# Atomu2014/deep-ctr

Hardware: AMD Instinct MI355X
Metric: examples/sec (higher is better)
Workload: dtype bf16; 1 GPU; FNN L3 train step: 16 fields, 937670 one-hot dims, k=10, hidden 300/100 tanh, batch 4096 per GPU, Zipf(1.1) ids; per_gpu_batch=4096, global_batch=4096, parallelism=single

## Files before the change

deep-ctr_amd/_capi.py:

```python
import ctypes as C
import os

_HERE = os.path.dirname(os.path.abspath(__file__))
LIB_PATH = os.environ.get("FNN_HIP_LIB") or os.path.join(_HERE, "libfnn_hip.so")

FNN_OK = 0
FNN_ERR_ARG, FNN_ERR_HIP, FNN_ERR_STATE, FNN_ERR_RANGE, FNN_ERR_NOMEM = -1, -2, -3, -4, -5
FNN_PREC_F32, FNN_PREC_BF16, FNN_PREC_BF16X3 = 0, 1, 2
PRECISIONS = {'f32': FNN_PREC_F32, 'bf16': FNN_PREC_BF16, 'bf16x3': FNN_PREC_BF16X3}
FNN_ACT_TANH, FNN_ACT_SIGMOID, FNN_ACT_LINEAR = 0, 1, 2
FNN_MEM_HOST, FNN_MEM_DEVICE = 0, 1
FNN_MODE_FM, FNN_MODE_BAG = 0, 1
FNN_DP_SPARSE_LOCAL, FNN_DP_SPARSE_EXCHANGE = 0, 1
FNN_DP_PAYLOAD_SLABS, FNN_DP_PAYLOAD_BUCKET = 0, 1
FNN_DP_COLLECTIVE_CALLBACK, FNN_DP_COLLECTIVE_P2P = 0, 1
ALLREDUCE_FN = C.CFUNCTYPE(C.c_int, C.c_void_p, C.c_void_p, C.c_int64, C.c_void_p)
ALLGATHER_FN = C.CFUNCTYPE(C.c_int, C.c_void_p, C.c_void_p, C.c_void_p, C.c_int64, C.c_void_p)


class fnn_cfg(C.Structure):
    _fields_ = [("n_fields", C.c_int32), ("k", C.c_int32), ("hidden1", C.c_int32),
                ("hidden2", C.c_int32), ("max_batch", C.c_int32), ("precision", C.c_int32),
                ("act", C.c_int32), ("reg_all", C.c_int32), ("lr", C.c_float),
                ("lambda1", C.c_float), ("lambda_fm", C.c_float), ("device", C.c_int32),
                ("stream", C.c_void_p), ("mode", C.c_int32), ("h0", C.c_int32)]


_vp, _i, _i64, _f = C.c_void_p, C.c_int, C.c_int64, C.c_float

SIGNATURES = {
    "fnn_version": (C.c_char_p, []),
    "fnn_cfg_size": (C.c_uint64, []),
    "fnn_last_error": (C.c_char_p, [_vp]),
    "fnn_scat1_form": (C.c_char_p, []),
    "fnn_scat2_form": (C.c_char_p, []),
    "fnn_create": (_i, [C.POINTER(fnn_cfg), C.POINTER(_vp)]),
    "fnn_destroy": (_i, [_vp]),
    "fnn_set_hparams": (_i, [_vp, _f, _f, _f]),
    "fnn_stream": (_vp, [_vp]),
    "fnn_sync": (_i, [_vp]),
    "fnn_set_table": (_i, [_vp, _vp, _i64, _vp, _f, _i]),
    "fnn_get_table": (_i, [_vp, _vp, _i]),
    "fnn_get_rows": (_i, [_vp, _vp, _i64, _vp, _i]),
    "fnn_set_dense": (_i, [_vp, _i, _vp, _vp, _i]),
    "fnn_get_dense": (_i, [_vp, _i, _vp, _vp, _i]),
    "fnn_set_bag_bias": (_i, [_vp, _vp, _i]),
    "fnn_get_bag_bias": (_i, [_vp, _vp, _i]),
    "fnn_gather": (_i, [_vp, _vp, _i, _vp, _i]),
    "fnn_train_step": (_i, [_vp, _vp, _vp, _i, _vp, _vp, _i, _vp, _vp, _i, C.POINTER(_f)]),
    "fnn_set_shadowed": (_i, [_vp, _vp, _i, _i]),
    "fnn_prefetch_ids": (_i, [_vp, _vp, _i]),
    "fnn_train_step_multi": (_i, [_vp, _i, _vp, _vp, _i, _vp, _vp, _i, _vp, _i, _vp, C.POINTER(_f)]),
    "fnn_dp_unique_id": (_i, [_vp]),
    "fnn_dp_init": (_i, [_vp, _i, _i, _vp, _i]),
    "fnn_dp_init_custom": (_i, [_vp, _i, _i, _vp, _vp, _vp, _i]),
    "fnn_dp_shutdown": (_i, [_vp]),
    "fnn_dp_set_payload": (_i, [_vp, _i]),
    "fnn_dp_p2p_export": (_i, [_vp, _vp, _i]),
    "fnn_dp_p2p_attach": (_i, [_vp, _vp, _i]),
    "fnn_dp_set_collective": (_i, [_vp, _i]),
    "fnn_dp_get_config": (_i, [_vp, C.POINTER(_i), C.POINTER(_i), C.POINTER(_i)]),
    "fnn_dp_p2p_max_wait_us": (_i, [_vp, C.POINTER(C.c_double)]),
    "fnn_step_begin": (_i, [_vp, _vp, _vp, _i, _vp, _vp, _i, _vp, _vp, _i]),
    "fnn_dense_grad_bucket": (_i, [_vp, C.POINTER(_vp), C.POINTER(_i64)]),
    "fnn_step_scatter": (_i, [_vp]),
    "fnn_sparse_grad": (_i, [_vp, C.POINTER(_vp), C.POINTER(_i64)]),
    "fnn_step_scatter_global": (_i, [_vp, _vp, _vp, _i]),
    "fnn_step_end": (_i, [_vp, C.POINTER(_f)]),
# ... 145 lines not shown
```

deep-ctr_amd/csrc/fm_api.hip:

```cpp
#include <hip/hip_runtime.h>

#include <algorithm>
#include <cmath>
#include <cstring>
#include <string>
#include <vector>

#include "../../include/fm_hip.h"
#include "../../include/fnn_hip.h"
#include "sparse_rows.hip.h"
#include "metrics.hip.h"
#include "optim.hip.h"
#include "fm_online.hip.h"
#include "arg_ring.h"

using namespace fnn;

namespace {

thread_local std::string g_fm_err;
inline int rup(int x, int m) { return (x + m - 1) / m * m; }

struct FmArgs {
    const int32_t* ids; const float* y; int B, F, K; const float* table16; int64_t n_rows; const float* b;
// ... 269 lines not shown
    fm_body<NF, WV>(a, (int)blockIdx.x - so.nblk, s_gb);
}

struct FmBiasOpt { int opt; float* sb; float lr, b1, b2, eps; };
__device__ __forceinline__ float fm_opt_step(int opt, float w, float g, float& s0, float& s1, float lr, float b1, float b2, float eps) {
    return opt == FM_OPT_FTRL ? ftrl_step(w, g, s0, s1, lr) : adam_step(w, g, s0, s1, lr, b1, b2, eps);
}

__device__ __forceinline__ void fm_tail_body(float* b, const float* gb_part, int n, float lr, float lambda, const float* loss_t, int Ba, float lscale,
                                             float* loss_out, float* sl, const FmBiasOpt& bo)
{
    float v = strided_sum256(gb_part, n);
    sl[threadIdx.x] = v; __syncthreads();
    for (int o = 128; o > 0; o >>= 1) { if ((int)threadIdx.x < o) sl[threadIdx.x] += sl[threadIdx.x + o]; __syncthreads(); }
    const float gsum = sl[0];
    __syncthreads();
    v = strided_sum256(loss_t, Ba);
    sl[threadIdx.x] = v; __syncthreads();
    for (int o = 128; o > 0; o >>= 1) { if ((int)threadIdx.x < o) sl[threadIdx.x] += sl[threadIdx.x + o]; __syncthreads(); }
    if (threadIdx.x == 0) {
        if (bo.opt) *b = fm_opt_step(bo.opt, *b, gsum + lambda * *b, bo.sb[0], bo.sb[1], bo.lr, bo.b1, bo.b2, bo.eps);
        else *b = *b * (1.0f - lr * lambda) - lr * gsum;
        *loss_out = sl[0] * lscale;
    }
}
__global__ __launch_bounds__(256) void k_fm_scat2_tail(const ScatArgs sa, float* b, const float* gb_part, int n, float lr, float lambda,
                                                       const float* loss_t, int Ba, float lscale, float* loss_out, const FmBiasOpt bo)
{
    __shared__ double s_sum[16][16];
    if (blockIdx.x == 0) { fm_tail_body(b, gb_part, n, lr, lambda, loss_t, Ba, lscale, loss_out, reinterpret_cast<float*>(&s_sum[0][0]), bo); return; }
    if (sa.form2 == SCAT2_WAVE) scat2w_body(sa, (int)blockIdx.x - 1, (int)gridDim.x - 1);
    else scat2_body(sa, (int)blockIdx.x - 1, (int)gridDim.x - 1, s_sum);
}
__global__ __launch_bounds__(256) void k_fm_scat1s(const ScatArgs sa) { scat1h_form<true>(sa, blockIdx.x); }
__global__ __launch_bounds__(256) void k_fm_scat2s_tail(const ScatArgs sa, float* b, const float* gb_part, int n, float lr, float lambda,
                                                        const float* loss_t, int Ba, float lscale, float* loss_out, const FmBiasOpt bo)
{
    __shared__ float s_l[256];
    if (blockIdx.x == 0) { fm_tail_body(b, gb_part, n, lr, lambda, loss_t, Ba, lscale, loss_out, s_l, bo); return; }
    scat2w_form<true>(sa, (int)blockIdx.x - 1, (int)gridDim.x - 1);
}
__global__ __launch_bounds__(256) void k_fm_count_marks(const int* __restrict__ tag_shared, int64_t n_rows, int stamp, unsigned long long* out)
{
    __shared__ int s_c[256];
    int c = 0;
    for (int64_t i = (int64_t)blockIdx.x * 256 + threadIdx.x; i < n_rows; i += (int64_t)gridDim.x * 256) c += tag_shared[i] == stamp;
    s_c[threadIdx.x] = c; __syncthreads();
    for (int o = 128; o > 0; o >>= 1) { if ((int)threadIdx.x < o) s_c[threadIdx.x] += s_c[threadIdx.x + o]; __syncthreads(); }
    if (threadIdx.x == 0 && s_c[0]) atomicAdd(out, (unsigned long long)s_c[0]);
}
__global__ __launch_bounds__(256) void k_fm_scatw1(const ScatArgs sa) { scatw1_body(sa, blockIdx.x); }
__global__ __launch_bounds__(256) void k_fm_scatw2_tail(const ScatArgs sa, float* b, const float* gb_part, int n, float lr, float lambda,
                                                        const float* loss_t, int Ba, float lscale, float* loss_out, const FmBiasOpt bo)
{
    __shared__ double s_w[1024];
    if (blockIdx.x == 0) { fm_tail_body(b, gb_part, n, lr, lambda, loss_t, Ba, lscale, loss_out, reinterpret_cast<float*>(s_w), bo); return; }
    scatw2_body(sa, (int)blockIdx.x - 1, (int)gridDim.x - 1, s_w);
}

struct StepTail { float* b; const float* gb_part; int n; float lr, lambda; const float* loss_t; int Ba; float lscale; float* loss_out; FmBiasOpt bo; };
struct StepPack { float loss; int flag; };
struct StepArg {
    FmArgs a; ScatArgs sa; StepTail t;
    int* own_marks; int own_stamp;
    StepPack* pack;
    int nb1;
    int fcls, scls;
    SortArgs so;
};
__device__ __forceinline__ void step_pick(const StepArg* __restrict__ args, const int ncls, const int mblk, const int first, const int tiles,
                                          int& m, int& tile)
{
    const int lin = (int)blockIdx.x - ncls * mblk;
    m = args[first + lin / tiles].fcls;
    tile = lin % tiles;
    if (tile == 0 && threadIdx.x == 0) *args[m].sa.owner_cnt = 0;
}
template <typename KT, int NF, bool WV>
__global__ __launch_bounds__(256) void k_fm_step_fwd(const StepArg* __restrict__ args, const int ncls, const int mblk, const int first,
                                                     const int tiles)
{
    extern __shared__ __align__(16) unsigned char smem[];
    __shared__ float s_gb[16];
    if ((int)blockIdx.x < ncls * mblk) { const SortArgs so = args[(int)blockIdx.x / mblk].so; sortB_body<KT>(so, (int)blockIdx.x % mblk, smem); return; }
    int m, tile;
    step_pick(args, ncls, mblk, first, tiles, m, tile);
    const FmArgs a = args[m].a;
    fm_body<NF, WV>(a, tile, s_gb);
}
template <typename KT, int L, int NC, bool WV>
__global__ __launch_bounds__(256) void k_fm_step_fwd_wide(const StepArg* __restrict__ args, const int ncls, const int mblk, const int first,
                                                          const int tiles)
{
    extern __shared__ __align__(16) unsigned char smem[];
    __shared__ float s_gb[256 / L];
    if ((int)blockIdx.x < ncls * mblk) { const SortArgs so = args[(int)blockIdx.x / mblk].so; sortB_body<KT>(so, (int)blockIdx.x % mblk, smem); return; }
    int m, tile;
    step_pick(args, ncls, mblk, first, tiles, m, tile);
    const FmArgs a = args[m].a;
    fm_wide_body<L, NC, WV>(a, tile, s_gb);
}
__device__ __forceinline__ void step_copy_marks(const StepArg& g, const ScatArgs& sa, const int blk, const int nblk)
{
    if (!g.own_marks) return;
    const int n = sa.F * sa.N2;
    for (int i = blk * 256 + (int)threadIdx.x; i < n; i += nblk * 256) {
        const int4 r = sa.rec[i];
        if (r.x >= 0 && (i % sa.N2) == r.z && sa.tag_shared[r.x] == sa.stamp) g.own_marks[r.x] = g.own_stamp;
    }
}
template <bool SHARED>
__global__ __launch_bounds__(256) void k_fm_step_scat1(const StepArg* __restrict__ args, const int first)
{
    const int m = args[first + blockIdx.y].scls;
    const int nb1 = args[m].nb1;
    if ((int)blockIdx.x >= nb1) return;
    const ScatArgs sa = args[m].sa;
    if (SHARED) step_copy_marks(args[m], sa, blockIdx.x, nb1);
    scat1h_form<SHARED>(sa, blockIdx.x);
}
__global__ __launch_bounds__(256) void k_fm_step_scatw1(const StepArg* __restrict__ args, const int first)
{
    const int m = args[first + blockIdx.y].scls;
    const int nb1 = args[m].nb1;
    if ((int)blockIdx.x >= nb1) return;
    const ScatArgs sa = args[m].sa;
    step_copy_marks(args[m], sa, blockIdx.x, nb1);
    scatw1_body(sa, blockIdx.x);
}
__device__ __forceinline__ void step_tail(const StepArg& g, float* sl)
{
    const StepTail t = g.t;
    fm_tail_body(t.b, t.gb_part, t.n, t.lr, t.lambda, t.loss_t, t.Ba, t.lscale, t.loss_out, sl, t.bo);
    if (threadIdx.x == 0 && g.pack) {
        const int flag = *static_cast<volatile int*>(g.a.err);
        g.pack->loss = *t.loss_out; g.pack->flag = flag;
        if (flag) *g.a.err = 0;
    }
}
template <bool SHARED>
__global__ __launch_bounds__(256) void k_fm_step_scat2_tail(const StepArg* __restrict__ args, const int first)
{
    __shared__ float s_l[256];
    const int m = args[first + blockIdx.y].scls;
    if (blockIdx.x == 0) { step_tail(args[m], s_l); return; }
    const ScatArgs sa = args[m].sa;
    scat2w_form<SHARED>(sa, (int)blockIdx.x - 1, (int)gridDim.x - 1);
}
__global__ __launch_bounds__(256) void k_fm_step_scatw2_tail(const StepArg* __restrict__ args, const int first)
{
    __shared__ double s_w[1024];
    const int m = args[first + blockIdx.y].scls;
    if (blockIdx.x == 0) { step_tail(args[m], reinterpret_cast<float*>(s_w)); return; }
    const ScatArgs sa = args[m].sa;
    scatw2_body(sa, (int)blockIdx.x - 1, (int)gridDim.x - 1, s_w);
}

__global__ void k_fm_rescale(float* table16, size_t n, float s)
{
    const size_t i = (size_t)blockIdx.x * blockDim.x + threadIdx.x;
    if (i < n) table16[i] *= s;
}

__global__ void k_fm_fill(float* p, size_t n, float v)
{
    const size_t i = (size_t)blockIdx.x * blockDim.x + threadIdx.x;
    if (i < n) p[i] = v;
}

template <bool DENSE_G>
__global__ __launch_bounds__(256) void k_fm_opt_pass(float* __restrict__ table16, float* __restrict__ G, const int* __restrict__ stamp, int step,
                                                     float* __restrict__ s0, float* __restrict__ s1, size_t nk, int K, int rw, float lambda,
                                                     int opt, float lr, float b1, float b2, float eps)
{
    const size_t e0 = ((size_t)blockIdx.x * blockDim.x + threadIdx.x) * 4;
    if (e0 >= nk) return;
    size_t row = e0 / K;
    int c = (int)(e0 - row * K);
    const float4 m4 = *reinterpret_cast<const float4*>(s0 + e0), v4 = *reinterpret_cast<const float4*>(s1 + e0);
    float m[4] = {m4.x, m4.y, m4.z, m4.w}, v[4] = {v4.x, v4.y, v4.z, v4.w}, w[4], g[4];
// ... 5 lines not shown
        off[j] = row * rw + c;
        w[j] = live[j] ? table16[off[j]] : 0.f;
        hit[j] = live[j] && (DENSE_G || stamp[row] == step);
        g[j] = hit[j] ? G[off[j]] : 0.f;
        if (++c == K) { c = 0; ++row; }
    }
#pragma unroll
    for (int j = 0; j < 4; ++j) {
        if (!live[j]) continue;
        w[j] = fm_opt_step(opt, w[j], g[j] + lambda * w[j], m[j], v[j], lr, b1, b2, eps);
        table16[off[j]] = w[j];
        if (hit[j]) G[off[j]] = 0.f;
    }
    *reinterpret_cast<float4*>(s0 + e0) = make_float4(m[0], m[1], m[2], m[3]);
    *reinterpret_cast<float4*>(s1 + e0) = make_float4(v[0], v[1], v[2], v[3]);
}


}

struct fm_handle {
    std::string err; int dev = 0; hipStream_t st = nullptr; bool own_stream = false;
    int F = 0, K = 0, Bmax = 0, K1p = 0;
    bool wide = false;
    int rw = SLOT;
    int* noshare = nullptr;
    float* table16 = nullptr; int64_t n_rows = 0; float* b = nullptr; double scale = 1.0;
    float *gxp = nullptr, *loss_t = nullptr, *gb_part = nullptr, *loss_dev = nullptr; int* err_flag = nullptr;
    RowGroupBufs rg; void* skeys = nullptr;
    double* cpow1 = nullptr; bool key64 = true;
    int opt = FM_OPT_SGD; float beta1 = 0.9f, beta2 = 0.999f, eps = 1e-8f; int64_t t = 0; bool dense_g = false;
    int scat_form = SCAT1_HALF;
    int scat2_form = SCAT2_WAVE;
    int sort_merge4 = 0;
    float *s0 = nullptr, *s1 = nullptr, *sb = nullptr, *G = nullptr; int* stamp = nullptr;
    bool shared = false; int* tag_first = nullptr; int* tag_shared = nullptr; int tag_stamp = 0, step_stamp = 0;
    unsigned long long* mark_cnt = nullptr;
    int64_t online_chunk = 65536; fm_online::Out* online_out = nullptr;
    ArgRing online_ring{sizeof(fm_online::Args), 8 * FM_ONLINE_MAX_MODELS};
    ArgRing step_ring{sizeof(StepArg), 4 * FM_STEP_MAX_MODELS};
    ArgRing eval_ring{sizeof(EvalArg), 4 * FM_EVAL_MAX_MODELS};
    hipEvent_t join = nullptr; StepPack* step_pack = nullptr;
};

#define MHK(h, expr) do { hipError_t e_ = (expr); if (e_ != hipSuccess) { (h)->err = std::string(#expr) + ": " + hipGetErrorString(e_); return FNN_ERR_HIP; } } while (0)
#define MFAIL(h, code, msg) do { (h)->err = (msg); return (code); } while (0)

namespace {

int fold_scale(fm_handle* h)
{
    if (h->scale == 1.0 || !h->table16) return FNN_OK;
    const size_t n = (size_t)h->n_rows * h->rw;
    hipLaunchKernelGGL(k_fm_rescale, dim3((unsigned)((n + 255) / 256)), dim3(256), 0, h->st, h->table16, n, (float)h->scale);
    MHK(h, hipGetLastError());
    h->scale = 1.0;
    return FNN_OK;
}

int alloc_tags(fm_handle* h)
{
    for (int** p : {&h->tag_first, &h->tag_shared}) { if (*p) hipFree(*p); *p = nullptr; }
    h->tag_stamp = h->step_stamp = 0;
    if (!h->shared || !h->table16) return FNN_OK;
    for (int** p : {&h->tag_first, &h->tag_shared}) {
        MHK(h, hipMalloc((void**)p, (size_t)h->n_rows * sizeof(int)));
// ... 135 lines not shown
    const int ex = h->wide ? wide_epb(h) : 16;
    launch_fwd<unsigned>(h, nullptr, predict_args(h, ids, wts, B, p_out, fm_wt_env()), rup(B, ex) / ex);
    MHK(h, hipGetLastError());
    return FNN_OK;
}

struct StepPlan { FmArgs a; ScatArgs sa; StepTail t; int nb1; float lr_step; };
StepPlan plan_step(fm_handle* h, const int32_t* ids, const float* wts, const float* y, int B, float lr, float lambda, int reduce_mean,
                   float* p_out, bool wt, const fm_handle* lead, int stamp, int form1, int form2)
{
    StepPlan p;
    const int F = h->F, ex = h->wide ? wide_epb(h) : 16, Ba = rup(B, ex);
    const bool opt = h->opt != FM_OPT_SGD;
    const float dscale = reduce_mean ? 1.0f / (float)B : 1.0f;
    p.lr_step = lr;
    if (opt) {
        h->t += 1;
        if (h->opt == FM_OPT_ADAM)
            p.lr_step = (float)((double)lr * std::sqrt(1.0 - std::pow((double)h->beta2, (double)h->t)) /
                                (1.0 - std::pow((double)h->beta1, (double)h->t)));
    }
    p.a = FmArgs{ids, y, B, F, h->K, h->table16, h->n_rows, h->b, (float)h->scale, dscale, 1, h->gxp, h->K1p, p_out, h->loss_t,
                 h->gb_part, h->err_flag, wt, opt && !h->dense_g ? h->stamp : nullptr, (int)h->t, h->rw, wts};
    if (!opt) h->scale *= 1.0 - (double)lr * (double)lambda;
    RowGroupBufs rg = h->rg;
    rg.rec = lead->rg.rec;
    p.sa = scat_args(rg, SORT_N, F, h->K, h->gxp, h->K1p, h->cpow1, opt ? -1.0 : (double)lr / h->scale, opt ? h->G : h->table16, h->rw);
    if (h->shared) { p.sa.tag_shared = lead->tag_shared; p.sa.stamp = stamp; }
    else if (h->wide) { p.sa.tag_shared = h->noshare; p.sa.stamp = 1; }
    if (h->wide) {
        p.sa.gxf = h->rw;
        p.nb1 = (F * (SORT_N / WCH) * (h->rw / 4) + 255) / 256;
    } else {
        p.nb1 = scat1_blocks(p.sa, form1);
        p.sa.form2 = form2;
    }
    p.t = StepTail{h->b, h->gb_part, Ba / ex, lr, lambda, h->loss_t, Ba, dscale, h->loss_dev,
                   opt ? FmBiasOpt{h->opt, h->sb, p.lr_step, h->beta1, h->beta2, h->eps} : FmBiasOpt{FM_OPT_SGD, nullptr, 0.f, 0.f, 0.f, 0.f}};
    return p;
}

int fm_step(fm_handle* h, const int32_t* ids, const float* wts, const float* y, int B, float lr, float lambda, int reduce_mean, float* p_out)
{
    const int F = h->F;
    SortArgs so{ids, B, F, h->n_rows, h->rg.rec, h->rg.owner_cnt, 4 * F, h->skeys};
    so.merge4 = h->sort_merge4;
    SortArgs sb = so; sb.nblk = 16 * F;
    set_claim(h, sb);
    const bool own_forms = !h->wide && !h->shared;
    const StepPlan p = plan_step(h, ids, wts, y, B, lr, lambda, reduce_mean, p_out, fm_wt_env(), h, sb.stamp,
                                 own_forms ? h->scat_form : SCAT1_HALF, own_forms ? h->scat2_form : SCAT2_WAVE);
    const StepTail& t = p.t;
    launch_sort_runs(h->st, h->key64, so);
    if (h->key64) launch_fwd<unsigned long long>(h, &sb, p.a, t.n);
    else launch_fwd<unsigned>(h, &sb, p.a, t.n);
#define FM_SCAT(k1, k2_tail) do { \
        hipLaunchKernelGGL(k1, dim3(p.nb1), dim3(256), 0, h->st, p.sa); \
        hipLaunchKernelGGL(k2_tail, dim3(1 + 256), dim3(256), 0, h->st, p.sa, t.b, t.gb_part, t.n, t.lr, t.lambda, t.loss_t, t.Ba, t.lscale, \
                           t.loss_out, t.bo); } while (0)
    if (h->wide) FM_SCAT(k_fm_scatw1, k_fm_scatw2_tail);
    else if (h->shared) FM_SCAT(k_fm_scat1s, k_fm_scat2s_tail);
    else FM_SCAT(k_scat1, k_fm_scat2_tail);
#undef FM_SCAT
    MHK(h, hipGetLastError());
    if (h->opt != FM_OPT_SGD) { launch_opt_pass(h, lambda, p.lr_step); MHK(h, hipGetLastError()); return FNN_OK; }
    if (h->scale < 5.96e-8 || h->scale > 1.0) return fold_scale(h);
    return FNN_OK;
}

void launch_opt_pass(fm_handle* h, float lambda, float lr_step)
{
    const size_t nk = (size_t)h->n_rows * h->K;
    const dim3 grid((unsigned)(((nk + 3) / 4 + 255) / 256));
    if (h->dense_g)
        hipLaunchKernelGGL(k_fm_opt_pass<true>, grid, dim3(256), 0, h->st, h->table16, h->G, h->stamp, (int)h->t, h->s0, h->s1, nk, h->K,
                           h->rw, lambda, h->opt, lr_step, h->beta1, h->beta2, h->eps);
    else
        hipLaunchKernelGGL(k_fm_opt_pass<false>, grid, dim3(256), 0, h->st, h->table16, h->G, h->stamp, (int)h->t, h->s0, h->s1, nk, h->K,
                           h->rw, lambda, h->opt, lr_step, h->beta1, h->beta2, h->eps);
}

int ring_take(fm_handle* h0, ArgRing& r, size_t n, size_t* slot)
{
    MHK(h0, fnn::ring_take(r, n, slot));
    return FNN_OK;
}
int ring_send(fm_handle* h0, ArgRing& r, size_t slot, size_t n)
{
    MHK(h0, fnn::ring_send(r, slot, n, h0->st));
    return FNN_OK;
}

struct GroupCall {
    const char* fn; fm_handle* const* hs; int n, max; fm_handle* h0;
// ... 63 lines not shown
int fm_create(int n_fields, int k, int max_batch, int device, void* stream, fm_handle** out)
{
    if (!out) { g_fm_err = "null argument"; return FNN_ERR_ARG; }
    *out = nullptr;
    if (n_fields < 1 || n_fields > 64 || k < 1 || k > 128 || max_batch < 1 || max_batch > SORT_N) {
        g_fm_err = "need 1 <= n_fields <= 64, 1 <= k <= 128 (rank 0..127), 1 <= max_batch <= 4096"; return FNN_ERR_ARG; }
    int ndev = 0;
    if (hipGetDeviceCount(&ndev) != hipSuccess || ndev <= 0) { g_fm_err = "no HIP device (libfnn_hip.so has no CPU fallback)"; return FNN_ERR_HIP; }
    fm_handle* h = new fm_handle();
    h->dev = device; h->F = n_fields; h->K = k; h->Bmax = max_batch;
    h->wide = k > 16; h->rw = h->wide ? rup(k, 4) : SLOT;
    h->K1p = h->wide ? n_fields * h->rw : rup(n_fields, 16) * SLOT;
    auto fail = [&](int code) { g_fm_err = h->err; fm_destroy(h); return code; };
#define FK(expr) do { hipError_t e2_ = (expr); if (e2_ != hipSuccess) { h->err = std::string(#expr) + ": " + hipGetErrorString(e2_); return fail(FNN_ERR_HIP); } } while (0)
    FK(hipSetDevice(h->dev));
    if (stream) h->st = (hipStream_t)stream; else { FK(hipStreamCreateWithFlags(&h->st, hipStreamNonBlocking)); h->own_stream = true; }
    auto al = [&](void** p, size_t bytes) { hipError_t e = hipMalloc(p, bytes); if (e == hipSuccess) e = hipMemsetAsync(*p, 0, bytes, h->st); return e; };
    const size_t Ba = rup(h->Bmax, 16);
    FK(al((void**)&h->gxp, Ba * h->K1p * 4)); FK(al((void**)&h->loss_t, Ba * 4)); FK(al((void**)&h->gb_part, (Ba / 8) * 4));
    FK(al((void**)&h->loss_dev, 4)); FK(al((void**)&h->b, 4)); FK(al((void**)&h->err_flag, 4)); FK(al((void**)&h->sb, 8));
    FK(al((void**)&h->mark_cnt, 8)); FK(al((void**)&h->online_out, sizeof(fm_online::Out)));
    FK(row_group_alloc(h->rg, h->F, SORT_N, h->wide, h->rw, h->st,  true));
    FK(al(&h->skeys, (size_t)h->F * SORT_N * 8));
    {
        std::vector<double> ones(SORT_N + 1, 1.0);
        FK(hipMalloc((void**)&h->cpow1, ones.size() * 8));
        FK(hipMemcpy(h->cpow1, ones.data(), ones.size() * 8, hipMemcpyHostToDevice));
    }
    FK(hipStreamSynchronize(h->st));
#undef FK
    h->dense_g = getenv("FM_OPT_DENSE_G") && atoi(getenv("FM_OPT_DENSE_G")) == 1;
    h->scat_form = scat1_form_env();
    h->scat2_form = scat2_form_env();
    h->sort_merge4 = sort_merge4_env(0);
    if (const char* e = getenv("FM_ONLINE_CHUNK")) { const long long c = atoll(e); if (c >= 1) h->online_chunk = c; }
    *out = h;
    return FNN_OK;
}

int fm_destroy(fm_handle* h)
{
    if (!h) return FNN_ERR_ARG;
    hipSetDevice(h->dev);
    if (h->st) hipStreamSynchronize(h->st);
    void* ptrs[] = {h->table16, h->b, h->gxp, h->loss_t, h->gb_part, h->loss_dev, h->err_flag, h->skeys, h->cpow1, h->s0, h->s1,
                    h->sb, h->G, h->stamp, h->noshare, h->tag_first, h->tag_shared, h->mark_cnt, h->online_out, h->step_pack};
    for (void* p : ptrs) if (p) hipFree(p);
    for (ArgRing* r : {&h->online_ring, &h->step_ring, &h->eval_ring}) ring_release(*r);
    if (h->join) hipEventDestroy(h->join);
    row_group_free(h->rg);
    if (h->own_stream && h->st) hipStreamDestroy(h->st);
    delete h;
    return FNN_OK;
}

int fm_sync(fm_handle* h)
{
    if (!h) return FNN_ERR_ARG;
    int flag = 0;
    MHK(h, hipMemcpyAsync(&flag, h->err_flag, 4, hipMemcpyDeviceToHost, h->st));
    MHK(h, hipStreamSynchronize(h->st));
    if (flag) { MHK(h, hipMemsetAsync(h->err_flag, 0, 4, h->st)); MFAIL(h, FNN_ERR_RANGE, "feature id outside [-1, n_rows)"); }
    return FNN_OK;
}

int fm_set_table(fm_handle* h, const float* rows, int64_t n_rows)
// ... 250 lines not shown
        if (c == (int)cls.size()) cls.push_back(Cls{hs[m], 0});
        cls_of[m] = c;
    }
    std::vector<int> order;
    for (int c = 0; c < (int)cls.size(); ++c) if (cls[c].lead->key64 == cls[0].lead->key64) order.push_back(c);
    const int nride = (int)order.size();
    for (int c = 0; c < (int)cls.size(); ++c) if (cls[c].lead->key64 != cls[0].lead->key64) order.push_back(c);
    std::vector<SortArgs> sorts(cls.size());
    for (int i = 0; i < (int)order.size(); ++i) {
        Cls& k = cls[order[i]];
        fm_handle* h = k.lead;
        SortArgs so{ids, B, F, h->n_rows, h->rg.rec, h->rg.owner_cnt, 4 * F, h->skeys};
        so.merge4 = h->sort_merge4;
        launch_sort_runs(st, h->key64, so);
        so.nblk = 16 * F;
        if (h->shared) {
            so.tag_first = h->tag_first; so.tag_shared = h->tag_shared;
            so.stamp = k.stamp = on_stream(h, st, [&] { return fm_next_stamp(h); });
        }
        sorts[i] = so;
        a[i].so = so;
    }
    MHK(h0, hipGetLastError());

    const bool wt = fm_wt_env();
    auto lay_of = [](const fm_handle* h) { return !h->wide ? 0 : h->rw <= 64 ? 1 : 2; };
    auto form_of = [](const fm_handle* h) { return h->wide ? 2 : h->shared ? 1 : 0; };
    int fcnt[3] = {0, 0, 0}, scnt[3] = {0, 0, 0}, ffirst[3], sfirst[3], fpos[3], spos[3], nb1max[3] = {0, 0, 0};
    for (int m = 0; m < M; ++m) { ++fcnt[lay_of(hs[m])]; ++scnt[form_of(hs[m])]; }
    ffirst[0] = sfirst[0] = 0;
    for (int c = 1; c < 3; ++c) { ffirst[c] = ffirst[c - 1] + fcnt[c - 1]; sfirst[c] = sfirst[c - 1] + scnt[c - 1]; }
    for (int c = 0; c < 3; ++c) { fpos[c] = ffirst[c]; spos[c] = sfirst[c]; }
    std::vector<float> lr_step(M);
    for (int m = 0; m < M; ++m) {
        fm_handle* h = hs[m];
        const Cls& k = cls[cls_of[m]];
        const StepPlan p = plan_step(h, ids, wts, y, B, lr[m], lambda[m], reduce_mean ? reduce_mean[m] : 0, p_out ? p_out[m] : nullptr, wt,
                                     k.lead, k.stamp, SCAT1_HALF, SCAT2_WAVE);
        a[m].a = p.a; a[m].sa = p.sa; a[m].t = p.t; a[m].nb1 = p.nb1;
        lr_step[m] = p.lr_step;
        a[m].own_marks = nullptr; a[m].own_stamp = 0;
        if (h->shared && h != k.lead) { a[m].own_marks = h->tag_shared; a[m].own_stamp = on_stream(h, st, [&] { return fm_next_stamp(h); }); }
        a[m].pack = pack ? pack + m : nullptr;
        a[fpos[lay_of(h)]++].fcls = m;
        a[spos[form_of(h)]++].scls = m;
        nb1max[form_of(h)] = std::max(nb1max[form_of(h)], p.nb1);
    }
    rc = ring_send(h0, h0->step_ring, slot, (size_t)M);
    if (rc != FNN_OK) return rc;
    for (int i = nride; i < (int)order.size(); ++i) {
        const SortArgs& so = sorts[i];
        if (cls[order[i]].lead->key64) hipLaunchKernelGGL((k_sortB<unsigned long long>), dim3(so.nblk), dim3(256), sort_lds_bytes<unsigned long long>(), st, so);
        else hipLaunchKernelGGL((k_sortB<unsigned>), dim3(so.nblk), dim3(256), sort_lds_bytes<unsigned>(), st, so);
    }
    int ride = nride;
    for (int c = 0; c < 3; ++c) {
        if (!fcnt[c]) continue;
        const int tiles = (B + (c == 2 ? 8 : 16) - 1) / (c == 2 ? 8 : 16);
        if (cls[0].lead->key64) launch_step_fwd<unsigned long long>(st, F, wts != nullptr, c, d, ride, 16 * F, ffirst[c], fcnt[c], tiles);
        else launch_step_fwd<unsigned>(st, F, wts != nullptr, c, d, ride, 16 * F, ffirst[c], fcnt[c], tiles);
        ride = 0;
    }
    MHK(h0, hipGetLastError());
    if (scnt[0]) hipLaunchKernelGGL(k_fm_step_scat1<false>, dim3(nb1max[0], scnt[0]), dim3(256), 0, st, d, sfirst[0]);
    if (scnt[1]) hipLaunchKernelGGL(k_fm_step_scat1<true>, dim3(nb1max[1], scnt[1]), dim3(256), 0, st, d, sfirst[1]);
    if (scnt[2]) hipLaunchKernelGGL(k_fm_step_scatw1, dim3(nb1max[2], scnt[2]), dim3(256), 0, st, d, sfirst[2]);
    if (scnt[0]) hipLaunchKernelGGL(k_fm_step_scat2_tail<false>, dim3(1 + 256, scnt[0]), dim3(256), 0, st, d, sfirst[0]);
    if (scnt[1]) hipLaunchKernelGGL(k_fm_step_scat2_tail<true>, dim3(1 + 256, scnt[1]), dim3(256), 0, st, d, sfirst[1]);
    if (scnt[2]) hipLaunchKernelGGL(k_fm_step_scatw2_tail, dim3(1 + 256, scnt[2]), dim3(256), 0, st, d, sfirst[2]);
    MHK(h0, hipGetLastError());
    for (int m = 0; m < M; ++m) {
        fm_handle* h = hs[m];
        if (h->opt != FM_OPT_SGD) {
            on_stream(h, st, [&] { launch_opt_pass(h, lambda[m], lr_step[m]); return 0; });
            MHK(h0, hipGetLastError());
        } else if (h->scale < 5.96e-8 || h->scale > 1.0) {
            const int rf = on_stream(h, st, [&] { return fold_scale(h); });
            if (rf != FNN_OK) return g.member_failed(rf, h, m);
        }
    }
    rc = g.leave();
    if (rc != FNN_OK || !loss_out) return rc;
    std::vector<StepPack> hp(M);
    MHK(h0, hipMemcpyAsync(hp.data(), pack, (size_t)M * sizeof(StepPack), hipMemcpyDeviceToHost, st));
    MHK(h0, hipStreamSynchronize(st));
    std::string bad;
    for (int m = 0; m < M; ++m) {
        loss_out[m] = hp[m].loss;
        if (hp[m].flag) bad += (bad.empty() ? "" : ", ") + std::to_string(m);
    }
    if (!bad.empty()) return g.refuse(FNN_ERR_RANGE, "feature id outside [-1, n_rows) in model(s) " + bad);
    return FNN_OK;
}

const char* fm_online_form(const fm_handle*) { return "plain"; }

int fm_predict(fm_handle* h, const int32_t* ids, int B, float* p_out) { return fm_predict_w(h, ids, nullptr, B, p_out); }

int fm_predict_w(fm_handle* h, const int32_t* ids, const float* wts, int B, float* p_out)
{
// ... 252 lines not shown
```

deep-ctr_amd/csrc/fnn_api.hip:

```cpp
#include <hip/hip_runtime.h>
#include <rccl/rccl.h>
#include <dlfcn.h>

#include <algorithm>

#include <cmath>
#include <cstdio>
#include <cstdlib>
#include <cstring>
#include <map>
#include <mutex>
#include <string>
#include <vector>

#include "../../include/fnn_hip.h"
#include "fnn_step_kernels.hip.h"
#include "metrics.hip.h"
#include "arg_ring.h"

using namespace fnn;

namespace {

thread_local std::string g_create_err;

struct ProfSlot { std::vector<std::pair<hipEvent_t, hipEvent_t>> ev; double ms = 0; int64_t n = 0; };

inline int rup(int x, int m) { return (x + m - 1) / m * m; }
constexpr int WIDE_XW_MAX = 4096;

struct FnnKnobs {
    int wt_stores = 47;
    int step1_waves = 8;
    bool step1_fixed = true;
    bool fused = true;
    int role_off = 0;
    int splitk = 0;
    int scat2_wgs = 256;
    int wgrad_form = -1;
    int scat_form = SCAT1_HALF;
    int scat2_form = SCAT2_WAVE;
    int sort_merge4 = 1;
};

template <typename... A> struct FnnKernel { void (*fn)(A...) = nullptr; int threads = 0; size_t lds = 0; };
template <typename T> using Step1Kernel = FnnKernel<MlpArgs<T>>;
using Step2Kernel = FnnKernel<SortArgs, WgradArgs, int, int, ScatArgs>;
using Step3Kernel = FnnKernel<SortArgs, TailArgs, ScatArgs>;
template <typename T> using GroupKernel = FnnKernel<const GroupArg<T>*>;
static_assert(sizeof(GroupArg<float>) == sizeof(GroupArg<bf16_t>) && sizeof(GroupArg<float>) == sizeof(GroupArg<bs16_t>), "one argument ring serves every element type");
template <typename T> using GroupPredKernel = FnnKernel<const GroupPredArg<T>*, int, int64_t, int, int64_t, int64_t, int>;
static_assert(sizeof(GroupPredArg<float>) == sizeof(GroupPredArg<bf16_t>) && sizeof(GroupPredArg<float>) == sizeof(GroupPredArg<bs16_t>), "one argument ring serves every element type");

struct FnnPlan {
    int F = 0, K = 0, H1 = 0, H2 = 0, xdim = 0, K1p = 0, H1p = 0, H2p = 0;
    int Bmax = 0, ldT = 0, N2max = 0;
    size_t n1 = 0, n2 = 0, nw12 = 0, nw = 0, nslab = 0;
    bool bf16 = false;
    bool split = false;
    bool bag = false; int rw = SLOT; size_t nbag = 0, off_bag = 0;
    bool wide = false;
    bool strip_shape = false;
    bool strip_ok = false;
    int three_launch_max_B = 0;
    int splitk = 4;
    int wgrad_lds = 0;
    FnnKernel<> step1[2];
    bool key64 = false;
    Step2Kernel step2[2];
    Step3Kernel step3[2];
};

}

// ... 142 lines not shown
}

bool strip_shape_ok(const FnnPlan& p) {
    if (p.wide) return false;
    const int c1 = p.H1p / 64, c2 = p.H2p / 64, cx = p.K1p / 64;
    if (cx == 5) return p.bag && c1 == 5 && c2 == 2;
    return cx == 4 && ((c1 == 5 && c2 == 2) || (c1 == 1 && c2 == 1));
}
int next_stamp(fnn_handle* h, fnn_handle::SortSlot& sl) {
    if (!h->bag) return 0;
    if (h->tag_stamp >= (1 << 25) - 1) {
        hipMemsetAsync(h->tag_first, 0, (size_t)h->n_rows * sizeof(int), h->st);
        for (auto& q : h->slot) hipMemsetAsync(q.tag_shared, 0, (size_t)h->n_rows * sizeof(int), h->st);
        h->tag_stamp = 0;
    }
    sl.stamp = ++h->tag_stamp;
    return sl.stamp;
}
int sort_n2(int B) { int N2 = 256; while (N2 < B) N2 <<= 1; return N2; }
constexpr int GLOBAL_BATCH_MAX = 32768;

template <typename T> WgradArgs make_wgrad_args(fnn_handle* h, int Ba) {
    WgradArgs wa;
    wa.p[0] = WgradProb{h->xpT, h->dl1T, h->slab, h->K1p / 64, h->H1p / 64, h->H1p};
    wa.p[1] = WgradProb{h->d1T, h->dl2T, h->slab + h->n1, h->H1p / 64, h->H2p / 64, h->H2p};
    wa.p[2] = WgradProb{h->d2T, h->dl3T, h->slab + h->nw12, h->H2p / 64, 1, 64};
    wa.p[3] = WgradProb{h->dlxT, h->onesT, h->slab + h->off_bag, h->bag ? h->K1p / 64 : 0, 1, 64};
    wa.ldT = h->ldT; wa.klen = Ba / h->splitk; wa.zstride = h->nslab;
    return wa;
}
int wgrad_blocks(const WgradArgs& wa) {
    return wa.p[0].mt * wa.p[0].nt + wa.p[1].mt * wa.p[1].nt + wa.p[2].mt * wa.p[2].nt + wa.p[3].mt * wa.p[3].nt;
}
ScatArgs make_scat_args(fnn_handle* h, const fnn_handle::SortSlot& sl, int N2) {
    ScatArgs sa = scat_args(sl, N2, h->F, h->K, h->gxp, h->K1p, h->cpow_dev, (double)h->cfg.lr, h->table16, h->rw);
    sa.tag_shared = sl.tag_shared; sa.stamp = sl.stamp; sa.form2 = h->kn.scat2_form;
    return sa;
}
template <typename T> MlpArgs<T> make_mlp_args(fnn_handle* h, const int32_t* ids, const float* y, int B,
                                                const uint8_t* m1, const uint8_t* m2, bool train, float* p_out) {
    return MlpArgs<T>{ids, y ? y : h->loss_t, B, h->F, h->K, h->table16, h->n_rows, h->w0,
                      (const T*)h->w1, (const T*)h->w1t, (const T*)h->w2, (const T*)h->w2t, h->master + h->nw12,
                      m1 ? m1 : h->ones_u8, m2 ? m2 : h->ones_u8, h->cfg.act, train ? ACT_TANH : h->cfg.act,
                      h->H1, h->H2, train ? 1 : 0,
                      (T*)h->xpT, (T*)h->d1T, (T*)h->d2T, (T*)h->dl1T, (T*)h->dl2T, (T*)h->dl3T, h->ldT,
                      h->gxp, p_out, h->loss_t, h->err_flag, h->bb0, h->rw, (T*)h->dlxT, nullptr, h->kn.wt_stores};
}
template <typename T> Step1Kernel<T> step1_sel(const FnnPlan& p, const FnnKnobs& kn, bool train)
{
#define STEP1(C1, C2, CX, BAG, NW, ...) Step1Kernel<T>{k_step1<T, C1, C2, CX, BAG, NW, ##__VA_ARGS__>, 64 * NW, mlp_lds_bytes<T, C1, C2, CX>(BAG, p.F, NW)}
    const bool big = p.H1p / 64 == 5, x5 = p.K1p / 64 == 5;
    if (big && kn.step1_waves == 8) {
        if (x5) return STEP1(5, 2, 5, true, 8);
        if (p.bag) return STEP1(5, 2, 4, true, 8);
        if constexpr (std::is_same<T, bf16_t>::value)
            if (kn.step1_fixed && train && kn.wt_stores == 47 && ((8 * p.F + 15) >> 4) * 32 <= 512) return STEP1(5, 2, 4, false, 8, 47);
        return STEP1(5, 2, 4, false, 8);
    }
    if (x5) return STEP1(5, 2, 5, true, 4);
    if (p.bag) return big ? STEP1(5, 2, 4, true, 4) : STEP1(1, 1, 4, true, 4);
    return big ? STEP1(5, 2, 4, false, 4) : STEP1(1, 1, 4, false, 4);
#undef STEP1
}
template <typename T> Step2Kernel step2_sel(bool key64, bool m4, bool wgrad_lds)
{
#define STEP2(WF) (key64 ? (m4 ? Step2Kernel{k_step2<T, unsigned long long, true, WF>, 256, lds} : Step2Kernel{k_step2<T, unsigned long long, false, WF>, 256, lds}) \
                         : (m4 ? Step2Kernel{k_step2<T, unsigned, true, WF>, 256, lds} : Step2Kernel{k_step2<T, unsigned, false, WF>, 256, lds}))
    const size_t lds = key64 ? sortA_lds_bytes<unsigned long long>(m4) : sortA_lds_bytes<unsigned>(m4);
    if constexpr (sizeof(T) == 2) if (wgrad_lds) return STEP2(WGRAD_LDS);
    return STEP2(WGRAD_DIRECT);
#undef STEP2
}
template <typename T> Step3Kernel step3_sel(bool key64, bool m4, bool update)
{
#define STEP3(KT, LDS) (m4 ? (update ? Step3Kernel{k_step3<T, true, KT, true>, 256, LDS} : Step3Kernel{k_step3<T, false, KT, true>, 256, LDS}) \
                           : (update ? Step3Kernel{k_step3<T, true, KT, false>, 256, LDS} : Step3Kernel{k_step3<T, false, KT, false>, 256, LDS}))
    return key64 ? STEP3(unsigned long long, sort_lds_bytes<unsigned long long>()) : STEP3(unsigned, sort_lds_bytes<unsigned>());
#undef STEP3
}
template <typename T> GroupKernel<T> gstep1_sel(const FnnPlan& p, const FnnKnobs& kn)
{
#define GSTEP1(C1, C2, NW, WTF) GroupKernel<T>{k_gstep1<T, C1, C2, 4, NW, WTF>, 64 * NW, mlp_lds_bytes<T, C1, C2, 4>(false, p.F, NW)}
    const bool big = p.H1p / 64 == 5;
    if (big && kn.step1_waves == 8) {
        if constexpr (std::is_same<T, bf16_t>::value)
            if (kn.step1_fixed && kn.wt_stores == 47 && ((8 * p.F + 15) >> 4) * 32 <= 512) return GSTEP1(5, 2, 8, 47);
        return GSTEP1(5, 2, 8, -1);
    }
    return big ? GSTEP1(5, 2, 4, -1) : GSTEP1(1, 1, 4, -1);
#undef GSTEP1
}
template <typename T> GroupPredKernel<T> gpredict_sel(const FnnPlan& p, const FnnKnobs& kn)
{
#define GPREDICT(C1, C2, NW) GroupPredKernel<T>{k_gpredict<T, C1, C2, 4, NW>, 64 * NW, mlp_lds_bytes<T, C1, C2, 4>(false, p.F, NW)}
    const bool big = p.H1p / 64 == 5;
    if (big && kn.step1_waves == 8) return GPREDICT(5, 2, 8);
    return big ? GPREDICT(5, 2, 4) : GPREDICT(1, 1, 4);
#undef GPREDICT
}
template <typename T> GroupKernel<T> gstep2_sel(bool key64, bool m4, bool wgrad_lds)
{
#define GSTEP2(WF) (key64 ? (m4 ? GroupKernel<T>{k_gstep2<T, unsigned long long, true, WF>, 256, lds} : GroupKernel<T>{k_gstep2<T, unsigned long long, false, WF>, 256, lds}) \
                          : (m4 ? GroupKernel<T>{k_gstep2<T, unsigned, true, WF>, 256, lds} : GroupKernel<T>{k_gstep2<T, unsigned, false, WF>, 256, lds}))
    const size_t lds = key64 ? sortA_lds_bytes<unsigned long long>(m4) : sortA_lds_bytes<unsigned>(m4);
    if constexpr (sizeof(T) == 2) if (wgrad_lds) return GSTEP2(WGRAD_LDS);
    return GSTEP2(WGRAD_DIRECT);
#undef GSTEP2
}
template <typename T> GroupKernel<T> gstep3_sel(bool key64, bool m4)
{
#define GSTEP3(KT) (m4 ? GroupKernel<T>{k_gstep3<T, KT, true>, 256, sort_lds_bytes<KT>()} : GroupKernel<T>{k_gstep3<T, KT, false>, 256, sort_lds_bytes<KT>()})
    return key64 ? GSTEP3(unsigned long long) : GSTEP3(unsigned);
#undef GSTEP3
}
template <typename T> void plan_step1(fnn_handle* h)
{
    for (int train = 0; train < 2; ++train) {
        const Step1Kernel<T> k = step1_sel<T>(*h, h->kn, train != 0);
        h->step1[train] = {reinterpret_cast<void (*)()>(k.fn), k.threads, k.lds};
    }
}
template <typename T> void plan_keys(fnn_handle* h, bool key64)
{
    h->key64 = key64;
    for (int i = 0; i < 2; ++i) {
        h->step2[i] = step2_sel<T>(key64, h->kn.sort_merge4 != 0, i && h->wgrad_lds);
        h->step3[i] = step3_sel<T>(key64, h->kn.sort_merge4 != 0, i != 0);
    }
}

template <typename T> void launch_step1(fnn_handle* h, int nmlp, const MlpArgs<T>& a) {
    const FnnKernel<>& k = h->step1[a.train];
    hipLaunchKernelGGL(reinterpret_cast<void (*)(MlpArgs<T>)>(k.fn), dim3(nmlp), dim3(k.threads), k.lds, h->st, a);
}
void launch_sort16(fnn_handle* h, SortArgs so) {
    so.merge4 = h->kn.sort_merge4;
    launch_sort(h->st, h->key64, so);
}

struct StepRoles { bool dense, sparse, group_next, update; const float* gxp_src; float* bucket_dst; };
StepRoles make_roles(const fnn_handle* h, bool dense, bool sparse, bool update, const float* gxp_src = nullptr, float* bucket_dst = nullptr)
{
    const int off = h->kn.role_off;
    return {dense && !(off & 2), sparse && !(off & 4), sparse && !(off & 1), update, gxp_src, bucket_dst};
}
struct Step23Args { bool have_next; ScatArgs sa; SortArgs so; };
Step23Args make_step23_args(fnn_handle* h, const StepRoles& r, bool merge)
{
    const bool have_next = r.group_next && h->pend_have_next;
    fnn_handle::SortSlot& nx = h->slot[h->cur ^ 1];
    Step23Args a{have_next, make_scat_args(h, h->slot[h->cur], SORT_N), {}};
    if (r.gxp_src) a.sa.gxp = r.gxp_src;
    a.so = SortArgs{h->next_ids, h->next_B, h->F, h->n_rows, nx.rec, nx.owner_cnt, have_next ? (merge ? 16 : 4) * h->F : 0, h->skeys,
                    merge ? h->tag_first : nullptr, merge ? nx.tag_shared : nullptr, merge && have_next ? next_stamp(h, nx) : 0, h->kn.sort_merge4};
    return a;
}
const char* role_name(const StepRoles& r, const char* both, const char* dense, const char* sparse) { return r.dense && r.sparse ? both : (r.dense ? dense : sparse); }

template <typename T> void launch_step2(fnn_handle* h, const StepRoles& r)
{
    Step23Args a = make_step23_args(h, r, false);
    ProfScope ps(h, role_name(r, "step2", "step2_dense", "step2_sparse"), h->st);
    const WgradArgs wa = make_wgrad_args<T>(h, h->pend_Ba);
    const int nwx = r.dense ? wgrad_blocks(wa) : 0;
    const int nsc = !r.sparse ? 0 : (h->bag ? (int)(((size_t)h->F * (SORT_N / WCH) * (h->rw / 4) + 255) / 256)
                                            : scat1_blocks(a.sa, h->kn.scat_form));
    const dim3 grid(a.so.nblk + nwx * h->splitk + nsc);
    if (grid.x == 0) return;
    const bool wl = nwx > 0 && h->wgrad_lds && sizeof(T) == 2;
    const Step2Kernel& k = h->step2[wl];
    hipLaunchKernelGGL(k.fn, grid, dim3(k.threads), std::max(k.lds, wl ? WGRAD_LDS_BYTES : (size_t)0), h->st, a.so, wa, nwx, h->splitk, a.sa);
}

TailArgs make_tail_args(const fnn_handle* h, const StepRoles& r)
{
    const int nred = r.dense ? (int)((h->nw12 / 4 + 255) / 256) + (int)((h->nw - h->nw12 + h->nbag + 255) / 256) + 1 : 0;
    return TailArgs{h->slab, h->splitk, h->nw, h->nw12, h->nslab, h->master, h->cfg.lambda1, h->cfg.reg_all,
                    h->loss_t, h->pend_Ba, r.bucket_dst ? r.bucket_dst : h->bucket, h->loss_dev, h->cfg.lr, h->K1p, h->H1p, h->H2p,
                    h->w1, h->w1t, h->w2, h->w2t, nred, h->bb0, h->nbag, h->off_bag};
}
void sparse_role_done(fnn_handle* h, bool have_next)
{
    if (have_next) { h->cur ^= 1; h->sorted_ids = h->next_ids; h->sorted_B = h->next_B; }
    else { h->sorted_ids = nullptr; h->sorted_B = 0; }
    h->next_ids = nullptr; h->next_B = 0;
// ... 175 lines not shown
    ProfScope ps(h, "gx", h->st);
    EpiF32 e{h->gxp, K1p, 0};
    launch_gemm<T, 4>(h->st, (T*)h->dl1, H1p, (const T*)h->w1, Ba, K1p, H1p, e);
}
template <typename T> int layers_wgrad_reduce(fnn_handle* h, int Ba)
{
    {
        ProfScope ps(h, "wgrad", h->st);
        const WgradArgs wa = make_wgrad_args<T>(h, Ba);
        const dim3 grid(wgrad_blocks(wa), h->splitk);
        bool lds_form = false;
        if constexpr (sizeof(T) == 2) {
            if (h->wgrad_lds) {
                hipLaunchKernelGGL((k_wgrad<T, WGRAD_LDS>), grid, dim3(256), WGRAD_LDS_BYTES, h->st, wa);
                lds_form = true;
            }
        }
        if (!lds_form) hipLaunchKernelGGL((k_wgrad<T>), grid, dim3(256), 0, h->st, wa);
    }
    if (h->step_native_dp && !dp_bucket_mode(h)) RCCHK(dp_allreduce(h, h->slab, (size_t)h->splitk * h->nslab, "weight-gradient slabs"));
    ProfScope ps(h, "reduce", h->st);
    hipLaunchKernelGGL(k_reduce, dim3((unsigned)((h->nw + 255) / 256 + 1)), dim3(256), 0, h->st, h->slab, h->splitk, h->nw, h->nw12,
                       h->nslab, h->master, h->cfg.lambda1, h->cfg.reg_all, h->loss_t, Ba, h->bucket, h->loss_dev);
    return FNN_OK;
}
void layers_row_update(fnn_handle* h, const fnn_handle::SortSlot& sl, int N2)
{
    ScatArgs sa = make_scat_args(h, sl, N2);
    if (h->wide) sa.gxf = h->rw;
    {
        ProfScope ps(h, "scatter", h->st);
        const int nblk = h->wide ? (int)(((size_t)h->F * (N2 / WCH) * (h->rw / 4) + 255) / 256) : scat1_blocks(sa, h->kn.scat_form);
        if (h->wide) hipLaunchKernelGGL(k_scatdw1, dim3(nblk), dim3(256), 0, h->st, sa);
        else hipLaunchKernelGGL(k_scat1, dim3(nblk), dim3(256), 0, h->st, sa);
    }
    ProfScope ps(h, "finalize", h->st);
    if (h->wide) hipLaunchKernelGGL(k_scatdw2, dim3(256), dim3(256), 0, h->st, sa);
    else hipLaunchKernelGGL(k_scat2, dim3(64), dim3(256), 0, h->st, sa);
}

template <typename T>
int run_step(fnn_handle* h, const int32_t* ids, const float* y, int B, const uint8_t* m1,
             const uint8_t* m2, bool train, float* p_out, float* gx_out_dev)
{
    const int Ba = rup(B, 256);
    const int nsh = train ? h->n_shadow : 0;
    const int N2 = sort_n2(B + nsh);
    if (nsh > 0) {
        if (B + nsh > 16384) FAIL(h, FNN_ERR_ARG, "batch plus shadowed features exceed 16384 keys per field");
        RCCHK(ensure_global_ws(h, B + nsh));
    }
    fnn_handle::SortSlot& sl = nsh > 0 ? h->gsl : h->slot[h->cur];
    h->sorted_ids = nullptr; h->next_ids = nullptr;
    if (h->bag && !h->strip_ok) FAIL(h, FNN_ERR_ARG, "FNN_MODE_BAG runs on the strip kernel only, which FNN_NO_FUSE=1 turns off (hidden1 256..319 with hidden2 64..127, or <= 63 / <= 63 at h0 <= 252)");
    if (h->bag && train) FAIL(h, FNN_ERR_ARG, "FNN_MODE_BAG trains through the three-launch path only (B <= 4096)");
    if (train && h->step_native_dp && h->dp_sparse == FNN_DP_SPARSE_EXCHANGE)
        FAIL(h, FNN_ERR_ARG, "FNN_DP_SPARSE_EXCHANGE runs on the three-launch path only (B <= 4096, hidden sizes the strip kernel is built for)");
    if (train) {
        ProfScope ps(h, "sort", h->st);
        launch_k_sort(h->st, N2, ids, B, h->F, h->n_rows, sl, h->shadow_dev, h->n_shadow, h->err_flag);
    }
    if (h->strip_ok) {
        ProfScope ps(h, "mlp", h->st);
        launch_step1<T>(h, Ba / 16, make_mlp_args<T>(h, ids, y, B, m1, m2, train, p_out));
    } else layers_forward<T>(h, ids, y, B, Ba, m1, m2, train, p_out);
    if (!train) return FNN_OK;
    if (!h->strip_ok) layers_backward<T>(h, B, Ba, m1);
    RCCHK(layers_wgrad_reduce<T>(h, Ba));
    if (gx_out_dev) copy_gx_out(h, B, gx_out_dev);
    layers_row_update(h, sl, N2);
    HIPCHK(h, hipGetLastError());
// ... 120 lines not shown
        RCCHK(alloc_dev(h, &h->xg_ids, rows * world * h->F));
        RCCHK(alloc_dev(h, &h->xg_gxp, rows * world * h->K1p));
        if (!h->bag) RCCHK(ensure_global_ws(h, (int)rows * world));
    }
    h->dp_rank = rank; h->dp_world = world; h->dp_sparse = sparse_mode;
    h->sorted_ids = nullptr; h->next_ids = nullptr;
    h->dp_payload = FNN_DP_PAYLOAD_SLABS; h->dp_collective = FNN_DP_COLLECTIVE_CALLBACK;
    if (const char* ev = getenv("FNN_DP_PAYLOAD")) {
        if (!strcmp(ev, "bucket")) h->dp_payload = FNN_DP_PAYLOAD_BUCKET;
        else if (strcmp(ev, "slabs") != 0) FAIL(h, FNN_ERR_ARG, "FNN_DP_PAYLOAD must be slabs or bucket");
    }
    return FNN_OK;
}

int check_ready(fnn_handle* h, int B) {
    if (!h) return FNN_ERR_ARG;
    if (B <= 0 || B > h->Bmax) FAIL(h, FNN_ERR_ARG, "B must be in [1, max_batch]");
    if (!h->table16) FAIL(h, FNN_ERR_STATE, "fnn_set_table has not been called");
    if (!(h->dense_set[0] && h->dense_set[1] && h->dense_set[2]))
        FAIL(h, FNN_ERR_STATE, "fnn_set_dense has not been called for all three layers");
    return FNN_OK;
}

FnnKnobs read_knobs(bool bag)
{
    FnnKnobs k;
    if (const char* e = getenv("FNN_WT_STORES")) k.wt_stores = atoi(e);
    if (const char* e = getenv("FNN_STEP1_WAVES")) k.step1_waves = atoi(e) == 4 ? 4 : 8;
    if (const char* e = getenv("FNN_STEP1_FORM")) k.step1_fixed = strcmp(e, "generic") != 0;
    if (const char* e = getenv("FNN_NO_FUSE")) k.fused = !(e[0] == '1');
    if (const char* e = getenv("FNN_ROLE_OFF")) k.role_off = atoi(e);
    if (const char* e = getenv("FNN_SPLITK")) { const int v = atoi(e); if (v == 2 || v == 4 || v == 8 || v == 16) k.splitk = v; }
    if (const char* e = getenv("FNN_SCAT2_WGS")) { const int v = atoi(e); if (v >= 16 && v <= 1024) k.scat2_wgs = v; }
    k.wgrad_form = wgrad_form_env(); k.scat_form = scat1_form_env(); k.scat2_form = scat2_form_env();
    k.sort_merge4 = sort_merge4_env(bag ? 0 : 1);
    return k;
}

FnnPlan make_plan(const fnn_cfg& c, const FnnKnobs& kn)
{
    FnnPlan p;
    p.F = c.n_fields; p.K = c.k; p.H1 = c.hidden1; p.H2 = c.hidden2;
    p.xdim = 1 + p.F * p.K;
    p.K1p = rup(p.F * SLOT, 64); p.H1p = rup(p.H1 + 1, 64); p.H2p = rup(p.H2 + 1, 64);
    p.bag = c.mode == FNN_MODE_BAG;
    if (p.bag) { p.rw = c.h0; p.K = c.h0; p.xdim = c.h0; p.K1p = rup(c.h0 + 1, 64); }
    p.wide = !p.bag && p.K >= 17;
    if (p.wide) { p.rw = rup(p.K, 4); p.K1p = rup(p.F * p.rw + 2, 64); }
    p.Bmax = c.max_batch; p.ldT = rup(p.Bmax, 256);
    p.N2max = SORT_N; while (p.N2max < p.Bmax) p.N2max <<= 1;
    p.n1 = (size_t)p.K1p * p.H1p; p.n2 = (size_t)p.H1p * p.H2p;
    p.nw12 = p.n1 + p.n2; p.nw = p.nw12 + p.H2p;
    p.off_bag = p.nw12 + (size_t)p.H2p * 64;
    p.nbag = p.bag ? (size_t)p.K1p : 0;
    p.nslab = p.off_bag + p.nbag * 64;
    p.bf16 = c.precision == FNN_PREC_BF16; p.split = c.precision == FNN_PREC_BF16X3;
    p.strip_shape = strip_shape_ok(p);
    p.strip_ok = kn.fused && p.strip_shape;
    p.three_launch_max_B = p.strip_ok ? SORT_N : 0;
    const bool eight = p.strip_ok && !p.bag && kn.scat_form != SCAT1_SLOT && !p.split && p.Bmax <= SORT_N;
    const bool lds_dflt = kn.wgrad_form == -1 && eight && p.bf16 && p.ldT / 4 / Traits<bf16_t>::KS >= WGRAD_LDS_S;
    p.wgrad_lds = kn.wgrad_form == WGRAD_LDS || lds_dflt ? 1 : 0;
    p.splitk = kn.splitk ? kn.splitk : (eight && !lds_dflt ? 8 : 4);
    return p;
}

struct StepGroup {
// ... 10 lines not shown
    {
        HIPCHK(h0, hipSetDevice(h0->dev));
        for (int m = 1; m < n; ++m) if (hs[m]->st != h0->st) others.push_back(hs[m]->st);
        std::sort(others.begin(), others.end());
        others.erase(std::unique(others.begin(), others.end()), others.end());
        if (!others.empty() && !h0->join) HIPCHK(h0, hipEventCreateWithFlags(&h0->join, hipEventDisableTiming));
        entered = true;
        for (hipStream_t o : others) {
            HIPCHK(h0, hipEventRecord(h0->join, o));
            HIPCHK(h0, hipStreamWaitEvent(h0->st, h0->join, 0));
        }
        return FNN_OK;
    }
    int leave()
    {
        if (!entered) return FNN_OK;
        entered = false;
        if (others.empty()) return FNN_OK;
        HIPCHK(h0, hipEventRecord(h0->join, h0->st));
        for (hipStream_t o : others) HIPCHK(h0, hipStreamWaitEvent(o, h0->join, 0));
        return FNN_OK;
    }
};
template <typename Fn> auto on_stream(fnn_handle* h, hipStream_t st, Fn fn)
{
    const hipStream_t own = h->st;
    h->st = st;
    auto r = fn();
    h->st = own;
    return r;
}

struct LaunchClass {
    FnnKernel<> k[3]; int prec, F, K, K1p, H1p, H2p, splitk, wl, scat_form, scat2_form, scat2_wgs, wt_stores, role_off;
    std::vector<int> members;
    bool same(const LaunchClass& o) const
    {
        for (int i = 0; i < 3; ++i) if (k[i].fn != o.k[i].fn || k[i].threads != o.k[i].threads || k[i].lds != o.k[i].lds) return false;
        return prec == o.prec && F == o.F && K == o.K && K1p == o.K1p && H1p == o.H1p && H2p == o.H2p && splitk == o.splitk && wl == o.wl &&
               scat_form == o.scat_form && scat2_form == o.scat2_form && scat2_wgs == o.scat2_wgs && wt_stores == o.wt_stores && role_off == o.role_off;
    }
};
template <typename T> LaunchClass launch_class_of(const fnn_handle* h)
{
    const bool m4 = h->kn.sort_merge4 != 0;
    const bool wl = !(h->kn.role_off & 2) && h->wgrad_lds && sizeof(T) == 2;
    const GroupKernel<T> k1 = gstep1_sel<T>(*h, h->kn), k2 = gstep2_sel<T>(h->key64, m4, wl), k3 = gstep3_sel<T>(h->key64, m4);
    LaunchClass c{};
    c.k[0] = {reinterpret_cast<void (*)()>(k1.fn), k1.threads, k1.lds};
    c.k[1] = {reinterpret_cast<void (*)()>(k2.fn), k2.threads, std::max(k2.lds, wl ? WGRAD_LDS_BYTES : (size_t)0)};
    c.k[2] = {reinterpret_cast<void (*)()>(k3.fn), k3.threads, k3.lds};
    c.prec = h->cfg.precision; c.F = h->F; c.K = h->K; c.K1p = h->K1p; c.H1p = h->H1p; c.H2p = h->H2p; c.splitk = h->splitk; c.wl = wl;
    c.scat_form = h->kn.scat_form; c.scat2_form = h->kn.scat2_form; c.scat2_wgs = h->kn.scat2_wgs; c.wt_stores = h->kn.wt_stores;
    c.role_off = h->kn.role_off;
    return c;
}
template <typename T>
bool fill_group_arg(fnn_handle* h, const int4* rec, const int32_t* ids, const float* y, int B, const uint8_t* m1, const uint8_t* m2,
                    float* p_out, GroupPack* pack, void* dst, int* x2, int* x3)
{
    GroupArg<T>& g = *static_cast<GroupArg<T>*>(dst);
    const StepRoles r = make_roles(h, true, true, true);
    g.ma = make_mlp_args<T>(h, ids, y, B, m1, m2, true, p_out);
    g.nmlp = h->pend_Ba / 16;
    Step23Args a = make_step23_args(h, r, false);
    a.sa.rec = rec;
    g.wa = make_wgrad_args<T>(h, h->pend_Ba);
    g.nwx = r.dense ? wgrad_blocks(g.wa) : 0; g.splitk = h->splitk;
    g.nsc1 = r.sparse ? scat1_blocks(a.sa, h->kn.scat_form) : 0;
    g.so2 = a.so; g.sa = a.sa;
    g.so3 = make_step23_args(h, r, true).so;
    g.ta = make_tail_args(h, r);
    g.nsc2 = r.sparse ? h->kn.scat2_wgs : 0;
    g.pack = pack;
    *x2 = g.so2.nblk + g.nwx * g.splitk + g.nsc1;
    *x3 = g.so3.nblk + g.ta.nblk_red + g.nsc2;
    return a.have_next;
}
template <typename T> void launch_group(const LaunchClass& c, hipStream_t st, const void* dev_args, int nmlp, int x2, int x3)
{
    const GroupArg<T>* d = static_cast<const GroupArg<T>*>(dev_args);
    const unsigned M = (unsigned)c.members.size();
    using Fn = void (*)(const GroupArg<T>*);
    hipLaunchKernelGGL(reinterpret_cast<Fn>(c.k[0].fn), dim3(nmlp, M), dim3(c.k[0].threads), c.k[0].lds, st, d);
    if (x2 > 0) hipLaunchKernelGGL(reinterpret_cast<Fn>(c.k[1].fn), dim3(rup(x2, 8), M), dim3(c.k[1].threads), c.k[1].lds, st, d);
    if (x3 > 0) hipLaunchKernelGGL(reinterpret_cast<Fn>(c.k[2].fn), dim3(x3, M), dim3(c.k[2].threads), c.k[2].lds, st, d);
// ... 117 lines not shown
        });
        if (rc != FNN_OK) { if (h != h0) g.refuse(rc, g.at(h->err, base + m)); return rc; }
    }
    *dev_args = reinterpret_cast<const GroupPredArg<float>*>(d);
    return FNN_OK;
}
int ensure_eval_y(fnn_handle* h0)
{
    if (h0->eval_y) return FNN_OK;
    HIPCHK(h0, hipMalloc((void**)&h0->eval_y, EVAL_FEED_BATCH_MAX * sizeof(float)));
    HIPCHK(h0, hipMemsetAsync(h0->eval_y, 0, EVAL_FEED_BATCH_MAX * sizeof(float), h0->st));
    return FNN_OK;
}
inline size_t up256(size_t b) { return (b + 255) / 256 * 256; }
size_t eval_scratch_bytes(int g, int64_t N)
{
    return up256((size_t)g * (size_t)N * 4) + up256(metrics_multi_bytes(g, N)) + up256((size_t)g * sizeof(MetricOut)) + up256((size_t)g * 4) + 256;
}

}

extern "C" {

const char* fnn_version(void) { return "fnn_hip 0.2 (gfx950)"; }

uint64_t fnn_cfg_size(void) { return (uint64_t)sizeof(fnn_cfg); }

const char* fnn_last_error(const fnn_handle* h) { return h ? h->err.c_str() : g_create_err.c_str(); }

const char* fnn_scat2_form(void)
{
    const int f = scat2_form_env(-1);
    return f == SCAT2_BLOCK ? "block" : f == SCAT2_WAVE ? "wave" : "default";
}

const char* fnn_scat1_form(void)
{
    const int f = scat1_form_env(-1);
    return f == SCAT1_SLOT ? "slot" : f == SCAT1_QUARTER ? "quarter" : f == SCAT1_HALF ? "half" : "default";
}

int fnn_create(const fnn_cfg* cfg, fnn_handle** out)
{
    if (!cfg || !out) { g_create_err = "null argument"; return FNN_ERR_ARG; }
    *out = nullptr;
    if (cfg->n_fields < 2 || cfg->n_fields > 64) { g_create_err = "n_fields must be in [2, 64]"; return FNN_ERR_ARG; }
    if (cfg->mode != FNN_MODE_FM && cfg->mode != FNN_MODE_BAG) { g_create_err = "bad mode"; return FNN_ERR_ARG; }
    if (cfg->mode == FNN_MODE_BAG && (cfg->h0 < 192 || cfg->h0 > 316 || cfg->h0 % 4 != 0)) {
        g_create_err = "FNN_MODE_BAG: h0 must be a multiple of 4 in [192, 316] (the strip kernel is built for bag rows of 256 or 320 padded floats; the reference uses 200 and 300, python/SNN_RBM.py:25,53)"; return FNN_ERR_ARG; }
    if (cfg->mode == FNN_MODE_FM && (cfg->k < 1 || cfg->k > 128 || cfg->k == 16)) {
        g_create_err = "k = rank+1 must be in [1, 15] (two pad slots of the 16-float row carry w_0 and the bias) or in [17, 128] (wide rows of rup(k, 4) floats); k = 16 is not supported"; return FNN_ERR_ARG; }
    if (cfg->mode == FNN_MODE_FM && cfg->k >= 17 && cfg->n_fields * rup(cfg->k, 4) > WIDE_XW_MAX) {
        g_create_err = "k >= 17: n_fields * rup(k, 4) must be <= 4096 (the layer-one width of the wide-row path)"; return FNN_ERR_ARG; }
    if (cfg->hidden1 < 1 || cfg->hidden1 > 4095 || cfg->hidden2 < 1 || cfg->hidden2 > 255) { g_create_err = "hidden1 must be in [1, 4095], hidden2 in [1, 255]"; return FNN_ERR_ARG; }
    if (cfg->max_batch < 1 || cfg->max_batch > 16384) { g_create_err = "max_batch must be in [1, 16384] (per-field LDS sort)"; return FNN_ERR_ARG; }
    if (cfg->precision != FNN_PREC_F32 && cfg->precision != FNN_PREC_BF16 && cfg->precision != FNN_PREC_BF16X3) { g_create_err = "bad precision"; return FNN_ERR_ARG; }
    if (cfg->act < 0 || cfg->act > 2) { g_create_err = "bad act"; return FNN_ERR_ARG; }
    const FnnKnobs kn = read_knobs(cfg->mode == FNN_MODE_BAG);
    if (kn.wgrad_form == -2) { g_create_err = "FNN_WGRAD_FORM must be direct or lds"; return FNN_ERR_ARG; }
    int ndev = 0;
    hipError_t e = hipGetDeviceCount(&ndev);
    if (e != hipSuccess || ndev <= 0) {
        g_create_err = std::string("no HIP device: ") + hipGetErrorString(e) + " (libfnn_hip.so has no CPU fallback)";
        return FNN_ERR_HIP;
    }
    if (cfg->device < 0 || cfg->device >= ndev) { g_create_err = "device ordinal out of range"; return FNN_ERR_ARG; }
// ... 962 lines not shown
```

deep-ctr_amd/csrc/fnn_step_kernels.hip.h:

```cpp
#pragma once
#include "fnn_kernels.hip.h"
#include "sparse_rows.hip.h"

namespace fnn {

template <typename T, int C1, int C2, int CX, bool BAG, int NW = 4, int WTF = -1>
static __global__ __launch_bounds__(64 * NW) void k_step1(const MlpArgs<T> a)
{
    extern __shared__ __align__(16) unsigned char smem[];
    mlp_body<T, C1, C2, CX, BAG, NW, WTF>(a, blockIdx.x, smem);
}

template <typename T, int WF>
__device__ __forceinline__ void wgrad_role(const WgradArgs& wa, const int nwx, int w, const int nw, const bool aligned, unsigned char* smem)
{
    if (aligned) {
        const int cls = w & 7, k = w >> 3, qd = nw >> 3, rm = nw & 7;
        w = (cls < rm ? cls * (qd + 1) : rm * (qd + 1) + (cls - rm) * qd) + k;
    }
    wgrad_body<T, WF>(wa, w % nwx, w / nwx, smem);
}
__device__ __forceinline__ void scat1_role(const ScatArgs& sa, const int blk)
{
    if (sa.rw != SLOT) scatw1_body(sa, blk);
    else if (sa.form == SCAT1_SLOT) scat1_body(sa, blk);
    else if (sa.form == SCAT1_HALF) scat1h_body(sa, blk);
    else scat1q_body(sa, blk);
}

template <typename T, typename KT, bool M4, int WF = WGRAD_DIRECT>
static __global__ __launch_bounds__(256) void k_step2(const SortArgs so, const WgradArgs wa, const int nwx,
                                               const int splitk, const ScatArgs sa)
{
    extern __shared__ __align__(16) unsigned char smem[];
    const int b = blockIdx.x, nw = nwx * splitk;
    if (b < so.nblk) sortA_form<KT, M4>(so, b, smem);
    else if (b < so.nblk + nw) {
        const int w = b - so.nblk;
        wgrad_role<T, WF>(wa, nwx, w, nw, ((b ^ w) & 7) == 0, smem);
    }
    else if (sa.rw != SLOT) scatw1_body(sa, b - so.nblk - nw);
    else if (sa.form == SCAT1_SLOT) scat1_body(sa, b - so.nblk - nw);
    else if (sa.form == SCAT1_HALF) scat1h_body(sa, b - so.nblk - nw);
    else scat1q_body(sa, b - so.nblk - nw);
}

struct TailArgs {
    const float* slab; int splitk; size_t nw_all, nw12, nslab; float* master; float lambda1; int reg_all;
    const float* loss_t; int Ba; float* bucket; float* loss_sum; float lr; int K1p, H1p, H2p;
    void *w1, *w1t, *w2, *w2t; int nblk_red;
    float* bb0; size_t nbag, off_bag;
};

template <typename T, bool UPDATE>
__device__ __forceinline__ void dense_body(const TailArgs& ta, const int b, double (&s_sum)[16][16])
{
    if (b == ta.nblk_red - 1) {
        float* s_l = reinterpret_cast<float*>(&s_sum[0][0]);
        float v = 0.f;
        v = strided_sum256(ta.loss_t, ta.Ba);
        s_l[threadIdx.x] = v;
        __syncthreads();
        for (int o = 128; o > 0; o >>= 1) {
            if ((int)threadIdx.x < o) s_l[threadIdx.x] += s_l[threadIdx.x + o];
            __syncthreads();
        }
        if (threadIdx.x == 0) *ta.loss_sum = s_l[0];
        return;
    }
    const size_t nvec = ta.nw12 / 4;
    const int nvb = (int)((nvec + 255) / 256);
    if (b < nvb) {
        const size_t q = (size_t)b * 256 + threadIdx.x;
        if (q >= nvec) return;
        const size_t i = q * 4;
// ... 15 lines not shown
            const size_t j = first ? i : i - n1;
            const int ld = first ? ta.H1p : ta.H2p, kin = first ? ta.K1p : ta.H1p;
            const int r = (int)(j / ld), c = (int)(j % ld);
            T* wn = static_cast<T*>(first ? ta.w1 : ta.w2);
            T* wt = static_cast<T*>(first ? ta.w1t : ta.w2t);
            store4(wn + ft_off<T>(r, c, ld), w.x, w.y, w.z, w.w);
            wt[ft_off<T>(c, r, kin)] = (T)w.x; wt[ft_off<T>(c + 1, r, kin)] = (T)w.y;
            wt[ft_off<T>(c + 2, r, kin)] = (T)w.z; wt[ft_off<T>(c + 3, r, kin)] = (T)w.w;
        }
        return;
    }
    const size_t i = ta.nw12 + (size_t)(b - nvb) * 256 + threadIdx.x;
    if (i >= ta.nw_all + ta.nbag) return;
    if (i >= ta.nw_all) {
        const size_t c = i - ta.nw_all;
        float g = 0.f;
#pragma unroll 8
        for (int z = 0; z < ta.splitk; ++z) g += ta.slab[(size_t)z * ta.nslab + ta.off_bag + c * 64];
        ta.bucket[i] = g;
        if (UPDATE) ta.bb0[c] -= ta.lr * g;
        return;
    }
    const size_t src = ta.nw12 + (i - ta.nw12) * 64;
    float g = 0.f;
#pragma unroll 8
    for (int z = 0; z < ta.splitk; ++z) g += ta.slab[(size_t)z * ta.nslab + src];
    float w = ta.master[i];
    ta.bucket[i] = g;
    if (UPDATE) {
        g += 2.0f * ta.lambda1 * w;
        ta.master[i] = w - ta.lr * g;
    }
}
__device__ __forceinline__ void scat2_role(const ScatArgs& sa, const int blk, const int nb, double (*s_sum)[16], unsigned char* smem)
{
    if (sa.rw == SLOT) {
        if (sa.form2 == SCAT2_WAVE) scat2w_body(sa, blk, nb);
        else scat2_body(sa, blk, nb, s_sum);
    }
    else scatw2_body(sa, blk, nb, reinterpret_cast<double*>(smem));
}

template <typename T, bool UPDATE, typename KT, bool M4>
static __global__ __launch_bounds__(256) void k_step3(const SortArgs so, const TailArgs ta, const ScatArgs sa)
{
    extern __shared__ __align__(16) unsigned char smem[];
    __shared__ double s_sum[16][16];
    if ((int)blockIdx.x < so.nblk) { sortB_form<KT, M4>(so, blockIdx.x, smem); return; }
    const int b = (int)blockIdx.x - so.nblk;
    if (b >= ta.nblk_red) {
        const int nb = (int)gridDim.x - so.nblk - ta.nblk_red;
        if (sa.rw == SLOT) {
            if (sa.form2 == SCAT2_WAVE) scat2w_body(sa, b - ta.nblk_red, nb);
            else scat2_body(sa, b - ta.nblk_red, nb, s_sum);
        }
        else scatw2_body(sa, b - ta.nblk_red, nb, reinterpret_cast<double*>(smem));
        return;
    }
    dense_body<T, UPDATE>(ta, b, s_sum);
}

struct GroupPack { float loss; int flag; };
template <typename T> struct GroupArg {
    MlpArgs<T> ma; int nmlp;
    SortArgs so2, so3;
    WgradArgs wa; int nwx, splitk, nsc1;
    ScatArgs sa;
    TailArgs ta; int nsc2;
    GroupPack* pack;
};

template <typename T, int C1, int C2, int CX, int NW, int WTF>
static __global__ __launch_bounds__(64 * NW) void k_gstep1(const GroupArg<T>* __restrict__ args)
{
    extern __shared__ __align__(16) unsigned char smem[];
    const GroupArg<T>& g = args[blockIdx.y];
    const MlpArgs<T> a = g.ma;
    const int nmlp = g.nmlp;
    int* const owner_cnt = g.sa.owner_cnt;
    if ((int)blockIdx.x >= nmlp) return;
    if (blockIdx.x == 0 && threadIdx.x == 0) *owner_cnt = 0;
    mlp_body<T, C1, C2, CX, false, NW, WTF>(a, blockIdx.x, smem);
}

template <typename T, typename KT, bool M4, int WF>
static __global__ __launch_bounds__(256) void k_gstep2(const GroupArg<T>* __restrict__ args)
{
    extern __shared__ __align__(16) unsigned char smem[];
    const GroupArg<T>& g = args[blockIdx.y];
    const int b = blockIdx.x, nsort = g.so2.nblk, nwx = g.nwx, nw = nwx * g.splitk, nsc = g.nsc1;
    if (b < nsort) { const SortArgs so = g.so2; sortA_form<KT, M4>(so, b, smem); }
    else if (b < nsort + nw) {
        const WgradArgs wa = g.wa;
        const int w = b - nsort;
        wgrad_role<T, WF>(wa, nwx, w, nw, ((b ^ w) & 7) == 0, smem);
    }
    else if (b < nsort + nw + nsc) { const ScatArgs sa = g.sa; scat1_role(sa, b - nsort - nw); }
}

template <typename T, typename KT, bool M4>
static __global__ __launch_bounds__(256) void k_gstep3(const GroupArg<T>* __restrict__ args)
{
    extern __shared__ __align__(16) unsigned char smem[];
    __shared__ double s_sum[16][16];
    const GroupArg<T>& g = args[blockIdx.y];
    const int nsort = g.so3.nblk, nred = g.ta.nblk_red, nsc = g.nsc2;
    if ((int)blockIdx.x < nsort) { const SortArgs so = g.so3; sortB_form<KT, M4>(so, blockIdx.x, smem); return; }
    const int b = (int)blockIdx.x - nsort;
    if (b >= nred) {
        if (b - nred < nsc) { const ScatArgs sa = g.sa; scat2_role(sa, b - nred, nsc, s_sum, smem); }
        return;
    }
    const TailArgs ta = g.ta;
    GroupPack* const pack = g.pack;
    int* const err = g.ma.err;
    dense_body<T, true>(ta, b, s_sum);
    if (pack && b == nred - 1 && threadIdx.x == 0) { pack->loss = *ta.loss_sum; pack->flag = *err; }
}

template <typename T> struct GroupPredArg { MlpArgs<T> ma; int m; };
template <typename T, int C1, int C2, int CX, int NW>
static __global__ __launch_bounds__(64 * NW) void k_gpredict(const GroupPredArg<T>* __restrict__ args, const int n_models, const int64_t N,
                                                             const int fb_len, const int64_t strip0, const int64_t n_strips, const int model_fast)
{
    extern __shared__ __align__(16) unsigned char smem[];
    int64_t s = blockIdx.x; int m = blockIdx.y;
    if (model_fast) {
        const int64_t l = (int64_t)blockIdx.y * gridDim.x + blockIdx.x;
        s = l / n_models; m = (int)(l % n_models);
    }
    if (s >= n_strips) return;
    s += strip0;
    MlpArgs<T> a = args[m].ma;
    const int per = fb_len >> 4;
    const int64_t lo = s / per * fb_len;
    a.ids += lo * a.F; a.p_out += lo;
    a.B = (int)(N - lo < fb_len ? N - lo : fb_len);
    mlp_body<T, C1, C2, CX, false, NW, -1>(a, (int)(s % per), smem);
}

struct P2PArgs {
    float* peer[8]; int world, rank; unsigned long long step; size_t bucket_off, flag_off; int* err;
    unsigned long long timeout_ticks;
// ... 69 lines not shown
```

deep-ctr_amd/csrc/ipnn_api.hip:

```cpp
#include <hip/hip_runtime.h>

#include <algorithm>
#include <cmath>
#include <cstring>
#include <map>
#include <string>
#include <vector>

#include "../../include/fnn_hip.h"
#include "../../include/ipnn_hip.h"
#include "fnn_kernels.hip.h"
#include "sparse_rows.hip.h"
#include "metrics.hip.h"
#include "optim.hip.h"

using namespace fnn;

namespace {

thread_local std::string g_ip_err;
inline int rup(int x, int m) { return (x + m - 1) / m * m; }

constexpr int A_TANH = IPNN_ACT_TANH, A_SIG = IPNN_ACT_SIGMOID, A_RELU = IPNN_ACT_RELU;

// ... 1302 lines not shown
        const int rl = r - r0;
        sT[cq][rl] = (T)w.x; sT[cq + 1][rl] = (T)w.y; sT[cq + 2][rl] = (T)w.z; sT[cq + 3][rl] = (T)w.w;
    }
    __syncthreads();
    T* wf = static_cast<T*>(u.wf[t]);
    for (int e = threadIdx.x; e < 64 * (64 / EPL); e += 256) {
        const int cl = e & 63, g8 = e >> 6;
        store16_sel(u.wt, wf + ft_off<T>(c0 + cl, r0 + g8 * EPL, Din), *reinterpret_cast<const frag*>(&sT[cl][g8 * EPL]));
    }
}

}

namespace {

struct IpKnobs {
    int side_stream = 1;
    int upd_side = 0;
    int mask_side = 0;
    int strip = 1;
    int gemm_lds = 0;
    int duo = 1, duo_min = DUO_MIN_BLOCKS;
    int tail_split = 1;
    int tail_fuse = 1;
    int tail_nf = 1, tail_nw = 16;
    int tail_w_lds = 0;
    int wide_nf = 2, wide_nw = 8;
    int strip_rot = 1, fwd_skip = 0;
    int strip_warm = 1;
    int ipf_nt = 1024;
    bool wt = true;
    int group_wgrad = 1, group_xcd = 1;
    int wgrad_want = 0;
    int scat_form = SCAT1_HALF, scat2_form = SCAT2_WAVE, sort_merge4 = 1;
    int stamps = 0, stamp_sel = -1;
};

struct IpEvents { hipEvent_t fork = nullptr, bwd = nullptr, wg = nullptr, join = nullptr, tab = nullptr, mask = nullptr; };

struct IpPlan {
    int maxD = 0; size_t strip_lds = 0;
    bool strip = false;
    bool pairs = false;
    int cut = 0, maxD2 = 0; size_t tail_lds = 0;
    size_t off[IPNN_MAX_HIDDEN + 2] = {};
    int wg_order[IPNN_MAX_HIDDEN + 1] = {};
    GemmGroupArgs group{};
    IpUpdArgs upd{};
    int mask_cols64[IPNN_MAX_HIDDEN + 1] = {};
};

}

struct ipnn_handle {
    ipnn_cfg cfg{}; std::string err; int dev = 0; hipStream_t st = nullptr; bool own_stream = false;
    int F = 0, K = 0, L = 0, P = 0, CB = 0, Bmax = 0, ldT = 0; bool bf16 = false; int splitk = 8;
    IpKnobs kn; IpPlan plan;
    bool wide = false;
    int rw = SLOT;
    int* noshare = nullptr;
    bool many_fwd = false, many_bwd = false;
    unsigned short* ptab = nullptr;
    std::vector<int> sk;
    bool adam = false; int64_t adam_t = 0;
    bool ftrl = false;
    bool loss_mean = false;
    std::vector<float*> Wm, Wv; float *tm = nullptr, *tv = nullptr, *tG = nullptr, *bmv = nullptr;
// ... 34 lines not shown
#define IRC(expr) do { const int rc_ = (expr); if (rc_ != FNN_OK) return rc_; } while (0)

namespace {

size_t ts(const ipnn_handle* h) { return h->bf16 ? 2 : 4; }

template <typename T> void ip_refresh(ipnn_handle* h, int t, const float* slab, float lr) {
    const int Din = h->Dp[t - 1], Dout = h->Dp[t];
    const size_t n = (size_t)Din * Dout;
    hipLaunchKernelGGL((k_ip_update<T>), dim3((unsigned)((n + 255) / 256)), dim3(256), 0, h->st, h->W[t - 1], slab, h->sk[t - 1],
                       h->slab_stride, lr, Din, Dout, (T*)h->wf[t - 1], (T*)h->wb[t - 1]);
}

inline int env_int(const char* name, int dflt) { const char* e = getenv(name); return e ? atoi(e) : dflt; }

IpKnobs ip_read_knobs()
{
    IpKnobs k;
    const struct { const char* name; int* v; bool flag; } plain[] = {
        {"IPNN_SIDE_STREAM", &k.side_stream, true}, {"IPNN_UPDATE_SIDE", &k.upd_side, true}, {"IPNN_MASK_SIDE", &k.mask_side, false},
        {"IPNN_STRIP", &k.strip, true}, {"IPNN_GEMM_LDS", &k.gemm_lds, true}, {"IPNN_STRIP_DUO", &k.duo, false}, {"IPNN_DUO_MIN", &k.duo_min, false},
        {"IPNN_TAIL_SPLIT", &k.tail_split, false}, {"IPNN_TAIL_FUSE", &k.tail_fuse, true}, {"IPNN_TAIL_LDS", &k.tail_w_lds, false},
        {"IPNN_STRIP_ROT", &k.strip_rot, false}, {"IPNN_FWD_SKIP", &k.fwd_skip, false}, {"IPNN_STRIP_WARM", &k.strip_warm, false},
        {"IPNN_GROUP_WGRAD", &k.group_wgrad, true}, {"IPNN_GROUP_XCD", &k.group_xcd, false}, {"IPNN_STAMP_SEL", &k.stamp_sel, false}};
    for (const auto& e : plain) { *e.v = env_int(e.name, *e.v); if (e.flag) *e.v = *e.v != 0; }
    k.wt = env_int("IPNN_WT", 1) != 0;
    k.duo_min = std::max(2, k.duo_min);
    { const int v = env_int("IPNN_TAIL_NF", 1); if (v == 1 || v == 2 || v == 4) k.tail_nf = v; }
    k.tail_nw = env_int("IPNN_TAIL_NW", 16) == 16 ? 16 : 8;
    k.ipf_nt = env_int("IPNN_IPF_NT", 1024) == 1024 ? 1024 : 512;
    int nf = 4, nw = 8;
    if (getenv("IPNN_WIDE") && sscanf(getenv("IPNN_WIDE"), "%d:%d", &nf, &nw) == 2 && ((nf == 2 && (nw == 8 || nw == 12)) || (nf == 4 && nw == 8))) { k.wide_nf = nf; k.wide_nw = nw; }
    k.wgrad_want = getenv("IPNN_WGRAD_WANT") ? std::max(16, env_int("IPNN_WGRAD_WANT", 0)) : k.group_wgrad ? 144 : 288;
    k.scat_form = scat1_form_env(); k.scat2_form = scat2_form_env(); k.sort_merge4 = sort_merge4_env(1);
    if (getenv("IPNN_STAMPS")) k.stamps = env_int("IPNN_STAMPS", 0) == 2 ? 2 : 1;
    return k;
}

int ip_join_table(ipnn_handle* h)
{
    if (h->tab_pending) { IHK(h, hipStreamWaitEvent(h->st, h->ev.tab, 0)); h->tab_pending = false; }
    return FNN_OK;
}
int ip_join(ipnn_handle* h)
{
    IRC(ip_join_table(h));
    if (h->upd_pending) { IHK(h, hipStreamWaitEvent(h->st, h->ev.join, 0)); h->upd_pending = false; }
    return FNN_OK;
}

struct IpSide {
    ipnn_handle* const h; hipStream_t const s; bool open = false;
    explicit IpSide(ipnn_handle* h_) : h(h_), s(h_->st2 ? h_->st2 : h_->st) {}
    IpSide(const IpSide&) = delete;
    bool on() const { return h->st2 != nullptr; }
    int fork(hipEvent_t ev)
    {
        if (!on()) return FNN_OK;
        IHK(h, hipEventRecord(ev, h->st));
        open = true;
        IHK(h, hipStreamWaitEvent(h->st2, ev, 0));
        return FNN_OK;
    }
    int signal(hipEvent_t ev) { if (on()) IHK(h, hipEventRecord(ev, h->st2)); return FNN_OK; }
    int wait(hipEvent_t ev) { if (on()) IHK(h, hipStreamWaitEvent(h->st, ev, 0)); return FNN_OK; }
    void settle() { open = false; }
    ~IpSide() { if (open && hipEventRecord(h->ev.join, h->st2) == hipSuccess) hipStreamWaitEvent(h->st, h->ev.join, 0); }
// ... 402 lines not shown
int ip_side_chain(ipnn_handle* h, const IpCall& c, hipStream_t ss, float lr_step)
{
    const int F = h->F;
    {
        IpProf ps(h, "ip_bwd", ss);
        const IpRows rows = ip_bwd_rows(h);
        const bool wv = c.wts != nullptr;
        const IpKernel k = ip_gather_bwd_sel(rows, wv);
        const float *dz0 = h->dz0, *emb = h->emb;
        if (rows == IP_WIDE) {
            const IpWideArgs wa = ip_wide_args(h, c, nullptr, 1.0f);
            IHK(h, ip_launch(k, c.Ba / IPW_EX, ipw_bwd_lds(F, h->rw, h->P, wv), ss, wa, dz0, emb, h->gxp, h->gb_part));
        } else if (rows == IP_MANY) {
            const IpManyArgs ma = ip_many_args(h, c, nullptr, 1.0f);
            IHK(h, ip_launch(k, c.Ba / IPM_BEX, ipm_bwd_lds(F, h->P, wv), ss, ma, dz0, emb, h->gxp, h->gb_part));
        } else {
            const IpBwdArgs ba{h->P, c.ids, c.B, F, h->K, h->table16, h->n_rows, h->Dp[0], h->emb, c.wts};
            IHK(h, ip_launch(k, c.Ba / 16, ip16_lds(F, h->Dp[0]), ss, ba, dz0, h->gxp, h->gb_part));
        }
        const int ngb = c.Ba / ip_bwd_ex(h);
        hipLaunchKernelGGL(k_ip_b_update, dim3(1), dim3(256), 0, ss, h->b, h->gb_part, ngb, h->adam ? (int)h->cfg.optimizer : 0, h->bmv,
                           lr_step, h->cfg.adam_beta1, h->cfg.adam_beta2, h->cfg.adam_eps, h->err_flag);
    }
    {
        IpProf ps(h, "scatter", ss);
        ScatArgs sa = scat_args(h->rg, SORT_N, F, h->K, h->gxp, h->Dp[0], h->cpow1, h->adam ? -1.0 : (double)h->cfg.lr,
                                h->adam ? h->tG : h->table16, h->wide ? h->rw : SLOT);
        if (h->wide) {
            sa.tag_shared = h->noshare; sa.stamp = 1; sa.gxf = h->rw;
            const int nthr = F * (SORT_N / WCH) * (h->rw / 4);
            hipLaunchKernelGGL(k_ip_scatw1, dim3((nthr + 255) / 256), dim3(256), 0, ss, sa);
            hipLaunchKernelGGL(k_ip_scatw2, dim3(256), dim3(256), 0, ss, sa);
        } else {
            sa.form2 = h->kn.scat2_form;
            launch_scat_narrow(ss, sa, h->kn.scat_form, 256);
        }
    }
    if (h->adam) {
        IpProf ps(h, "adam_table", ss);
        const size_t n = (size_t)h->n_rows * h->rw;
        hipLaunchKernelGGL(k_adam_table, dim3((unsigned)((n / 4 + 255) / 256)), dim3(256), 0, ss, h->table16, h->tm, h->tv, h->tG, n,
                           lr_step, h->cfg.adam_beta1, h->cfg.adam_beta2, h->cfg.adam_eps, (int)h->cfg.optimizer);
    }
    return FNN_OK;
}

template <typename T> void ip_wgrad(ipnn_handle* h, const IpCall& c)
{
    IpProf ps(h, "wgrad");
    const IpPlan& p = h->plan;
    const int L = h->L;
    constexpr int KS = Traits<T>::KS;
    if (h->kn.group_wgrad && L + 1 <= GEMM_GROUP_MAX) {
        GemmGroupArgs g = p.group;
        for (int i = 0; i <= L; ++i) g.p[i].nkt = c.Ba / KS / h->sk[p.wg_order[i] - 1];
        hipLaunchKernelGGL((k_gemm_group<T, 4, 4>), dim3(g.wg0[L + 1]), dim3(256), gemm_f32w_lds(), h->st, g);
        return;
    }
    for (int t = 1; t <= L + 1; ++t) {
        const int sk = h->sk[t - 1];
        ip_gemm(h, (const T*)h->aT[t - 1], (const T*)h->dlT[t - 1], h->Dp[t - 1], h->Dp[t], h->ldT / KS, c.Ba / KS / sk, sk,
                EpiF32{h->slab + p.off[t - 1], h->Dp[t], h->slab_stride});
    }
}

template <typename T> void ip_dense_update(ipnn_handle* h, const IpCall& c, hipStream_t us, float lr_step)
{
// ... 491 lines not shown
```

deep-ctr_amd/csrc/metrics.hip:

```cpp
#include "metrics.hip.h"

#include <cstring>
#include <rocprim/device/device_radix_sort.hpp>

#include <cmath>
#include <vector>

namespace fnn {
namespace {

constexpr int MB = 256;
constexpr int ITEMS = 8;

__device__ __forceinline__ void metric_keys_body(const float* __restrict__ p, const int32_t* __restrict__ y, int64_t n,
                                                 uint32_t* __restrict__ keys, double* __restrict__ part ,
                                                 unsigned long long* __restrict__ cnt_pos, unsigned long long* __restrict__ cnt_bad)
{
    __shared__ double s_se[MB], s_ll[MB];
    __shared__ unsigned s_np;
    if (threadIdx.x == 0) s_np = 0;
    __syncthreads();
    const double eps = 2.220446049250313e-16;
    double se = 0.0, ll = 0.0; unsigned np_ = 0;
    const int64_t base = (int64_t)blockIdx.x * MB * ITEMS;
// ... 156 lines not shown
#pragma unroll
    for (int k = 0; k < RS_ITEMS; ++k) {
        const bool valid = base + k * 64 + lane < n;
        const unsigned d = (unsigned)(key[k] >> shift) & 255u;
        unsigned long long m = __ballot(valid);
#pragma unroll
        for (int b = 0; b < 8; ++b) { const unsigned long long bb = __ballot((d >> b) & 1u); m &= ((d >> b) & 1u) ? bb : ~bb; }
        const unsigned before = s_cnt[wave][d];
        pre[k] = before + (unsigned)__popcll(m & lt);
        if (valid && (m & lt) == 0ull) s_cnt[wave][d] = before + (unsigned)__popcll(m);
    }
    __syncthreads();
    {
        unsigned run = 0;
#pragma unroll
        for (int w = 0; w < 4; ++w) { const unsigned c = s_cnt[w][tid]; s_cnt[w][tid] = run; run += c; }
    }
    __syncthreads();
#pragma unroll
    for (int k = 0; k < RS_ITEMS; ++k) {
        if (base + k * 64 + lane >= n) continue;
        const unsigned d = (unsigned)(key[k] >> shift) & 255u;
        out[s_base[d] + s_cnt[wave][d] + pre[k]] = key[k];
    }
}

constexpr int G_TB = 20, G_RB = 31;
constexpr unsigned long long G_INV = (1ull << G_RB) - 1;

__global__ __launch_bounds__(256) void k_group_keys(const int32_t* __restrict__ ids, int B, int F, int64_t n_rows, int N2,
                                                    unsigned long long* __restrict__ keys, int* __restrict__ owner_cnt)
{
    const size_t gid = (size_t)blockIdx.x * 256 + threadIdx.x;
    if (gid == 0) *owner_cnt = 0;
    if (gid >= (size_t)F * N2) return;
    const int f = (int)(gid / N2), t = (int)(gid % N2);
    unsigned long long row = G_INV;
    if (t < B) {
        const int64_t id = ids[(size_t)t * F + f];
        if (id >= 0 && id < n_rows) row = (unsigned long long)id;
    }
    keys[gid] = ((unsigned long long)f << (G_RB + G_TB)) | (row << G_TB) | (unsigned long long)t;
}

__global__ __launch_bounds__(256) void k_group_rec(const unsigned long long* __restrict__ sorted, int F, int N2, int4* __restrict__ rec)
{
    const size_t gid = (size_t)blockIdx.x * 256 + threadIdx.x;
    if (gid >= (size_t)F * N2) return;
    const int f = (int)(gid / N2), pos = (int)(gid % N2);
    const unsigned long long key = sorted[gid];
    const unsigned long long row = (key >> G_TB) & G_INV;
    int4 r = make_int4(-1, 0, 0, 0);
    if (row != G_INV) {
        const unsigned long long* q = sorted + (size_t)f * N2;
        const unsigned long long lo_key = key & ~((1ull << G_TB) - 1), hi_key = lo_key + (1ull << G_TB);
        int lo = 0, hi = pos;
        while (lo < hi) { const int mid = (lo + hi) >> 1; if (q[mid] < lo_key) lo = mid + 1; else hi = mid; }
        const int s = lo;
        lo = pos + 1; hi = N2;
        while (lo < hi) { const int mid = (lo + hi) >> 1; if (q[mid] < hi_key) lo = mid + 1; else hi = mid; }
        r = make_int4((int)row, (int)(key & ((1ull << G_TB) - 1)), s, lo);
    }
    rec[gid] = r;
}

}

// ... 137 lines not shown
```

deep-ctr_amd/csrc/metrics.hip.h:

```cpp
#pragma once
#include <hip/hip_runtime.h>
#include <stdint.h>
#include <string>

namespace fnn {
int device_metrics(hipStream_t st, const float* p, const int32_t* y, int64_t n, double out[4], std::string& err);

int group_global(hipStream_t st, const int32_t* ids, int B, int F, int64_t n_rows, int N2, int4* rec, int* owner_cnt,
                 void** ws, size_t* ws_bytes, std::string& err);

unsigned long long* radix_sort_segments(hipStream_t st, unsigned long long* keys, unsigned long long* tmp, unsigned* hist, int nseg, int n,
                                        int lo_bit, int hi_bit);
size_t radix_sort_hist_bytes(int nseg, int n);
uint32_t* radix_sort_segments32(hipStream_t st, uint32_t* keys, uint32_t* tmp, unsigned* hist, int nseg, int n, int lo_bit, int hi_bit);

struct MetricOut { double se, ll; unsigned long long auc_sum, n_bad; };
size_t metrics_multi_bytes(int nseg, int64_t n);
hipError_t metrics_multi(hipStream_t st, const float* p, const int32_t* y, int64_t n, int nseg, void* scratch, int count_pos,
                         unsigned long long* n_pos, MetricOut* out);
constexpr int GROUP_INDEX_BITS = 20;
constexpr unsigned long long GROUP_INVALID_ROW = (1ull << 31) - 1;
void group_records(hipStream_t st, const unsigned long long* sorted, int nseg, int n, int4* rec);
}
```

deep-ctr_amd/csrc/sparse_rows.hip.h:

```cpp
#pragma once
#include "fnn_kernels.hip.h"

namespace fnn {

template <typename KT> struct KeyTraits;
template <> struct KeyTraits<unsigned> { static constexpr int SH = 12; };
template <> struct KeyTraits<unsigned long long> { static constexpr int SH = 32; };

struct SortArgs {
    const int32_t* ids; int B, F; int64_t n_rows; int4* rec; int* owner_cnt; int nblk; void* skeys;
    int* tag_first; int* tag_shared; int stamp;
    int merge4;
};

constexpr int SORT_N = 4096;

template <typename KT> __host__ __device__ constexpr size_t sort_lds_bytes() { return (size_t)SORT_N * sizeof(KT); }
template <typename KT> inline size_t sortA_lds_bytes(const int merge4) { return merge4 ? (size_t)1024 * sizeof(KT) : 0; }
inline int sort_merge4_env(const int dflt)
{
    const char* e = getenv("FNN_SORT_RUNS");
    const int v = e ? atoi(e) : 0;
    return v == 16 ? 0 : (v == 4 ? 1 : dflt);
}

template <typename KT> __device__ __forceinline__ KT inv_row() { return (~(KT)0) >> KeyTraits<KT>::SH; }

template <typename KT, int LOG>
__device__ __forceinline__ int lower_bound_pow2(const KT* q, const KT v) {
    int base = 0;
#pragma unroll
    for (int s = 1 << (LOG - 1); s >= 1; s >>= 1) base += (q[base + s - 1] < v) ? s : 0;
    return base + ((q[base] < v) ? 1 : 0);
}

template <typename KT, bool M4>
__device__ __forceinline__ void sortA_form(const SortArgs& so, const int blk, unsigned char* smem)
{
    constexpr int SH = KeyTraits<KT>::SH;
    const int tid = threadIdx.x, wave = tid >> 6, lane = tid & 63, F = so.F, B = so.B;
// ... 52 lines not shown
            for (int a = 0; a < 4; ++a) bq[o][a] = ((wave + 1 + o) & 3) * 256;
#pragma unroll
        for (int st = 128; st >= 1; st >>= 1)
#pragma unroll
            for (int o = 0; o < 3; ++o)
#pragma unroll
                for (int a = 0; a < 4; ++a) bq[o][a] += s_run[bq[o][a] + st - 1] < key[a] ? st : 0;
#pragma unroll
        for (int o = 0; o < 3; ++o)
#pragma unroll
            for (int a = 0; a < 4; ++a)
                place[a] += bq[o][a] - ((wave + 1 + o) & 3) * 256 + (s_run[bq[o][a]] < key[a] ? 1 : 0);
        KT* out = static_cast<KT*>(so.skeys) + (size_t)f * SORT_N + (blk & 3) * 1024;
#pragma unroll
        for (int a = 0; a < 4; ++a) out[place[a]] = key[a];
        return;
    }
    KT* out = static_cast<KT*>(so.skeys) + (size_t)f * SORT_N + base + i0;
#pragma unroll
    for (int a = 0; a < 4; ++a) out[a] = key[a];
}
template <typename KT>
__device__ __forceinline__ void sortA_body(const SortArgs& so, const int blk, unsigned char* smem)
{
    if (so.merge4) sortA_form<KT, true>(so, blk, smem); else sortA_form<KT, false>(so, blk, smem);
}

template <typename KT, bool M4>
__device__ __forceinline__ void sortB_form(const SortArgs& so, const int blk, unsigned char* smem)
{
    constexpr int SH = KeyTraits<KT>::SH;
    KT* s_key = reinterpret_cast<KT*>(smem);
    const int tid = threadIdx.x, f = blk >> 4, run = blk & 15;
    if (blk == 0 && tid == 0) *so.owner_cnt = 0;
    const KT* in = static_cast<const KT*>(so.skeys) + (size_t)f * SORT_N;
#pragma unroll
    for (int a = 0; a < 16; ++a) s_key[a * 256 + tid] = in[a * 256 + tid];
    __syncthreads();
    const KT key = s_key[run * 256 + tid];
    const KT row = key >> SH, lo_key = row << SH, hi_key = (row + 1) << SH;
    int pos = 0, s = 0, e = 0;
    if constexpr (M4) {
        const int own = run >> 2;
        int bp[3], bs[4], be[4];
#pragma unroll
        for (int o = 0; o < 3; ++o) bp[o] = ((own + 1 + o) & 3) * 1024;
#pragma unroll
        for (int r = 0; r < 4; ++r) bs[r] = be[r] = r * 1024;
#pragma unroll
        for (int st = 512; st >= 1; st >>= 1) {
#pragma unroll
            for (int o = 0; o < 3; ++o) bp[o] += s_key[bp[o] + st - 1] < key ? st : 0;
#pragma unroll
            for (int r = 0; r < 4; ++r) {
                const KT vs = s_key[bs[r] + st - 1], ve = s_key[be[r] + st - 1];
                bs[r] += vs < lo_key ? st : 0; be[r] += ve < hi_key ? st : 0;
            }
        }
        pos = (run & 3) * 256 + tid;
#pragma unroll
        for (int o = 0; o < 3; ++o) pos += bp[o] - ((own + 1 + o) & 3) * 1024 + (s_key[bp[o]] < key ? 1 : 0);
#pragma unroll
        for (int r = 0; r < 4; ++r) {
            s += bs[r] - r * 1024 + (s_key[bs[r]] < lo_key ? 1 : 0);
            e += be[r] - r * 1024 + (s_key[be[r]] < hi_key ? 1 : 0);
        }
    } else {
// ... 24 lines not shown
            if ((old >> 6) == so.stamp && old != mine) so.tag_shared[(size_t)row] = so.stamp;
        }
    }
    so.rec[(size_t)f * SORT_N + pos] = rr;
}
template <typename KT>
__device__ __forceinline__ void sortB_body(const SortArgs& so, const int blk, unsigned char* smem)
{
    if (so.merge4) sortB_form<KT, true>(so, blk, smem); else sortB_form<KT, false>(so, blk, smem);
}

template <typename KT>
static __global__ __launch_bounds__(256) void k_sortA(const SortArgs so)
{
    extern __shared__ __align__(16) unsigned char smem[];
    sortA_body<KT>(so, blockIdx.x, smem);
}
template <typename KT>
static __global__ __launch_bounds__(256) void k_sortB(const SortArgs so)
{
    extern __shared__ __align__(16) unsigned char smem[];
    sortB_body<KT>(so, blockIdx.x, smem);
}

template <int KPT>
static __global__ __launch_bounds__(1024) void k_sort(const int32_t* __restrict__ ids, int B, int F,
                                               int64_t n_rows, int N2, int4* __restrict__ rec,
                                               int* __restrict__ owner_cnt, const int32_t* __restrict__ extra, int n_extra,
                                               int* __restrict__ err)
{
    extern __shared__ unsigned long long s_key[];
    __shared__ int s_cnt;
    const int f = blockIdx.x, tid = threadIdx.x;
    if (f == 0 && tid == 0) *owner_cnt = 0;
    int cnt = 0;
    if (n_extra > 0) {
        if (tid == 0) s_cnt = 0;
        __syncthreads();
        for (int j = tid; j < n_extra; j += blockDim.x) {
            const int t = extra[3 * j], ff = extra[3 * j + 1]; const int64_t r = extra[3 * j + 2];
            if (ff < 0 || ff >= F || t < 0 || t >= B || r < 0 || r >= n_rows) { if (f == 0) atomicOr(err, 1); continue; }
            if (ff != f) continue;
            const int p = atomicAdd(&s_cnt, 1);
            if (B + p < N2) s_key[B + p] = ((unsigned long long)r << 32) | (unsigned)t;
        }
        __syncthreads();
        cnt = min(s_cnt, N2 - B);
    }
    unsigned long long key[KPT];
#pragma unroll
    for (int a = 0; a < KPT; ++a) {
        const int i = tid * KPT + a;
        unsigned long long kk = ~0ull;
        if (i < B) {
            const int64_t id = ids[(size_t)i * F + f];
            if (id >= 0 && id < n_rows) kk = ((unsigned long long)id << 32) | (unsigned)i;
        } else if (i < B + cnt) kk = s_key[i];
        key[a] = kk;
    }
    if (n_extra > 0) __syncthreads();
    for (int k = 2; k <= N2; k <<= 1) {
        for (int j = k >> 1; j > 0; j >>= 1) {
            if (j < KPT) {
#pragma unroll
                for (int jj = KPT >> 1; jj > 0; jj >>= 1) {
                    if (j == jj) {
#pragma unroll
// ... 34 lines not shown
        }
    }
    __syncthreads();
#pragma unroll
    for (int a = 0; a < KPT; ++a) s_key[tid * KPT + a] = key[a];
    __syncthreads();
#pragma unroll
    for (int a = 0; a < KPT; ++a) {
        const int pos = tid * KPT + a;
        const unsigned long long kk = key[a];
        int4 r = make_int4(-1, 0, 0, 0);
        if (kk != ~0ull) {
            const unsigned long long lo_key = kk & 0xffffffff00000000ull;
            const unsigned long long hi_key = lo_key + 0x100000000ull;
            int lo = 0, hi = pos;
            while (lo < hi) { const int mid = (lo + hi) >> 1; if (s_key[mid] < lo_key) lo = mid + 1; else hi = mid; }
            const int s = lo;
            lo = pos + 1; hi = N2;
            while (lo < hi) { const int mid = (lo + hi) >> 1; if (s_key[mid] < hi_key) lo = mid + 1; else hi = mid; }
            r = make_int4((int)(kk >> 32), (int)(kk & 0xffffffffu), s, lo);
        }
        rec[(size_t)f * N2 + pos] = r;
    }
}

struct ScatArgs {
    const int4* rec; int N2, F, K; const float* gxp; int K1p; const double* cpow; double lr;
    float* table16; double* part; int* owner_cnt; int4* owners;
    int rw;
    const int* tag_shared; int stamp;
    int gxf;
    int form;
    int form2;
};
enum { SCAT1_QUARTER = 0, SCAT1_SLOT = 1, SCAT1_HALF = 2 };
__device__ __forceinline__ void atomic_add4(float* p, float a, float b, float c, float d) {
    atomicAdd(p, a); atomicAdd(p + 1, b); atomicAdd(p + 2, c); atomicAdd(p + 3, d);
}
__device__ __forceinline__ void scat1_body(const ScatArgs& sa, const int blk)
{
    const int4* __restrict__ rec = sa.rec; const int N2 = sa.N2, F = sa.F, K = sa.K, K1p = sa.K1p;
    const float* __restrict__ gxp = sa.gxp; const double* __restrict__ cpow = sa.cpow; const double lr = sa.lr;
    float* __restrict__ table16 = sa.table16; double* __restrict__ part = sa.part;
    int* __restrict__ owner_cnt = sa.owner_cnt; int4* __restrict__ owners = sa.owners;
    const int l = threadIdx.x & 15;
    const int G = (blk * 256 + threadIdx.x) >> 4;
    const int NQ = N2 >> 4;
    if (G >= F * NQ) return;
    const int f = G / NQ, q = G % NQ, base = q * 16;
    const int4 mine = rec[(size_t)f * N2 + base + l];
    const double wmine = (mine.x >= 0) ? cpow[mine.w - 1 - (base + l)] : 0.0;
    const double cmine = (mine.x >= 0) ? cpow[mine.w - mine.z] : 0.0;
    int row[16], sg[16], eg[16];
    float g[16], wold[16];
    double w[16], cs[16];
#pragma unroll
    for (int j = 0; j < 16; ++j) {
        row[j] = __shfl(mine.x, j, 16);
        const int t = __shfl(mine.y, j, 16);
        sg[j] = __shfl(mine.z, j, 16);
        eg[j] = __shfl(mine.w, j, 16);
        w[j] = __shfl(wmine, j, 16);
        cs[j] = __shfl(cmine, j, 16);
        const bool live = row[j] >= 0 && l < K;
        g[j] = live ? gxp[(size_t)t * K1p + f * SLOT + l] : 0.f;
        wold[j] = live ? table16[(size_t)row[j] * SLOT + l] : 0.f;
    }
// ... 61 lines not shown
#pragma unroll
        for (int j = 0; j < 8; ++j) {
            if (r[j].x < 0) continue;
            a0 += (double)g[j].x * wd[j]; a1 += (double)g[j].y * wd[j]; a2 += (double)g[j].z * wd[j]; a3 += (double)g[j].w * wd[j];
            const int pos = base + sb + j, s = r[j].z, e = r[j].w;
            if (pos + 1 != e && pos + 1 != base + 16) continue;
            if (s >= base && e <= base + 16) {
                float4 o = make_float4((float)((double)wold[j].x * cs[j] - lr * a0), (float)((double)wold[j].y * cs[j] - lr * a1),
                                       (float)((double)wold[j].z * cs[j] - lr * a2), (float)((double)wold[j].w * cs[j] - lr * a3));
                if (lim < 4) {
                    if (lim < 2) o.y = wold[j].y;
                    if (lim < 3) o.z = wold[j].z;
                    o.w = wold[j].w;
                }
                *reinterpret_cast<float4*>(sa.table16 + (size_t)r[j].x * SLOT + 4 * q) = o;
            } else {
                const int which = (s < base) ? 0 : 1;
                double* pp = sa.part + (((size_t)f * NQ + qc) * 2 + which) * SLOT + 4 * q;
                pp[0] = a0; pp[1] = a1; pp[2] = a2; pp[3] = a3;
                if (which == 1 && q == 0) sa.owners[atomicAdd(sa.owner_cnt, 1)] = make_int4(f, s, e, r[j].x);
            }
            a0 = a1 = a2 = a3 = 0;
        }
    }
}

__device__ __forceinline__ double lane_below(const double v)
{
    const int lo = __builtin_amdgcn_update_dpp(0, __double2loint(v), 0xA0, 0xf, 0xf, false);
    const int hi = __builtin_amdgcn_update_dpp(0, __double2hiint(v), 0xA0, 0xf, 0xf, false);
    return __hiloint2double(hi, lo);
}

template <bool SHARED>
__device__ __forceinline__ void scat1h_form(const ScatArgs& sa, const int blk)
{
    const int N2 = sa.N2, NQ = N2 >> 4, nq = (sa.K + 3) >> 2;
    const int gid = blk * 256 + (int)threadIdx.x;
    const int half = gid & 1, cq = gid >> 1;
    const int chunk = cq / nq, q = cq % nq;
    if (chunk >= sa.F * NQ) return;
    const int f = chunk / NQ, qc = chunk % NQ, base = qc * 16, hb = base + 8 * half;
    const int lim = sa.K - 4 * q;
    const double* __restrict__ cpow = sa.cpow; const double lr = sa.lr;
    int4 r[8];
#pragma unroll
    for (int j = 0; j < 8; ++j) r[j] = sa.rec[(size_t)f * N2 + hb + j];
    float4 g[8], wold[8];
    double wd[8], cs[8];
    int mk[8];
#pragma unroll
    for (int j = 0; j < 8; ++j) {
        const int pos = hb + j;
        const bool live = r[j].x >= 0;
        g[j] = *reinterpret_cast<const float4*>(sa.gxp + (size_t)(live ? r[j].y : 0) * sa.K1p + f * SLOT + 4 * q);
        const bool need = live && pos + 1 == r[j].w && r[j].z >= base;
        wold[j] = *reinterpret_cast<const float4*>(sa.table16 + (size_t)(need ? r[j].x : 0) * SLOT + 4 * q);
        wd[j] = cpow[live ? r[j].w - 1 - pos : 0];
        cs[j] = cpow[need ? r[j].w - r[j].z : 0];
        if (SHARED) mk[j] = sa.tag_shared[need ? r[j].x : 0];
    }
    if (lim < 4) {
#pragma unroll
        for (int j = 0; j < 8; ++j) {
            if (lim < 2) g[j].y = 0.f;
            if (lim < 3) g[j].z = 0.f;
            g[j].w = 0.f;
        }
    }
    double a0 = 0, a1 = 0, a2 = 0, a3 = 0;
#pragma unroll
    for (int j = 0; j < 8; ++j) {
        if (r[j].x < 0) continue;
        a0 += (double)g[j].x * wd[j]; a1 += (double)g[j].y * wd[j]; a2 += (double)g[j].z * wd[j]; a3 += (double)g[j].w * wd[j];
        if (hb + j + 1 == r[j].w) a0 = a1 = a2 = a3 = 0;
    }
    a0 = lane_below(a0); a1 = lane_below(a1); a2 = lane_below(a2); a3 = lane_below(a3);
    if (!half) a0 = a1 = a2 = a3 = 0;
#pragma unroll
    for (int j = 0; j < 8; ++j) {
        if (r[j].x < 0) continue;
        a0 += (double)g[j].x * wd[j]; a1 += (double)g[j].y * wd[j]; a2 += (double)g[j].z * wd[j]; a3 += (double)g[j].w * wd[j];
        const int pos = hb + j, s = r[j].z, e = r[j].w;
        if (pos + 1 != e && pos + 1 != base + 16) continue;
        if (SHARED && s >= base && e <= base + 16 && mk[j] == sa.stamp) {
            atomic_add4(sa.table16 + (size_t)r[j].x * SLOT + 4 * q, (float)(-lr * a0), (float)(-lr * a1), (float)(-lr * a2), (float)(-lr * a3));
        } else if (s >= base && e <= base + 16) {
            float4 o = make_float4((float)((double)wold[j].x * cs[j] - lr * a0), (float)((double)wold[j].y * cs[j] - lr * a1),
                                   (float)((double)wold[j].z * cs[j] - lr * a2), (float)((double)wold[j].w * cs[j] - lr * a3));
            if (lim < 4) {
                if (lim < 2) o.y = wold[j].y;
                if (lim < 3) o.z = wold[j].z;
                o.w = wold[j].w;
            }
            *reinterpret_cast<float4*>(sa.table16 + (size_t)r[j].x * SLOT + 4 * q) = o;
        } else {
            const int which = (s < base) ? 0 : 1;
            double* pp = sa.part + (((size_t)f * NQ + qc) * 2 + which) * SLOT + 4 * q;
            pp[0] = a0; pp[1] = a1; pp[2] = a2; pp[3] = a3;
            if (which == 1 && q == 0) sa.owners[atomicAdd(sa.owner_cnt, 1)] = make_int4(f, s, e, r[j].x);
        }
        a0 = a1 = a2 = a3 = 0;
    }
}
__device__ __forceinline__ void scat1h_body(const ScatArgs& sa, const int blk) { scat1h_form<false>(sa, blk); }

static __global__ __launch_bounds__(256) void k_scat1(const ScatArgs sa)
{
    if (sa.form == SCAT1_SLOT) scat1_body(sa, blockIdx.x);
    else if (sa.form == SCAT1_HALF) scat1h_body(sa, blockIdx.x);
    else scat1q_body(sa, blockIdx.x);
}

inline int scat1_blocks(ScatArgs& sa, const int form)
{
    const bool vec_ok = ((uintptr_t)sa.gxp | (uintptr_t)sa.table16) % 16 == 0 && sa.K1p % 4 == 0;
    sa.form = vec_ok ? form : SCAT1_SLOT;
    const size_t nquarters = (size_t)sa.F * (sa.N2 / 16) * ((sa.K + 3) / 4);
    const size_t nthr = sa.form == SCAT1_SLOT ? (size_t)sa.F * sa.N2 : sa.form == SCAT1_HALF ? 2 * nquarters : nquarters;
    return (int)((nthr + 255) / 256);
}
inline int scat1_form_env(const int dflt = SCAT1_HALF)
{
    const char* e = getenv("FNN_SCAT1_FORM");
    if (!e) return dflt;
    return !strcmp(e, "slot") ? SCAT1_SLOT : !strcmp(e, "quarter") ? SCAT1_QUARTER : !strcmp(e, "half") ? SCAT1_HALF : dflt;
}

__device__ __forceinline__ void scat2_body(const ScatArgs& sa, const int blk, const int nblk, double (*s_sum)[16])
{
    const int4* __restrict__ owners = sa.owners; const int N2 = sa.N2, K = sa.K;
    const double* __restrict__ part = sa.part; const double* __restrict__ cpow = sa.cpow; const double lr = sa.lr;
    float* __restrict__ table16 = sa.table16;
    const int n = *sa.owner_cnt;
    const int l = threadIdx.x & 15, grp = threadIdx.x >> 4;
    const int NQ = N2 >> 4;
    for (int o = blk; o < n; o += nblk) {
        const int4 ow = owners[o];
        const int q0 = ow.y >> 4, q1 = (ow.z - 1) >> 4;
        double sum = 0.0;
        float* p = table16 + (size_t)ow.w * SLOT + l;
        float wold = 0.f; double cdec = 0.0;
        if (grp == 0 && l < K) { wold = *p; cdec = cpow[ow.z - ow.y]; }
        for (int qb = q0 + grp; qb <= q1; qb += 64) {
            double v[4];
#pragma unroll
            for (int k = 0; k < 4; ++k) {
                const int q = qb + 16 * k;
                v[k] = q <= q1 ? part[(((size_t)ow.x * NQ + q) * 2 + (q == q0 ? 1 : 0)) * SLOT + l] : 0.0;
            }
// ... 9 lines not shown
            *p = (float)((double)wold * cdec - lr * tot);
        }
        __syncthreads();
    }
}

__device__ __forceinline__ double lane_from(const double v, const int src)
{
    const int lo = __shfl(__double2loint(v), src, 64), hi = __shfl(__double2hiint(v), src, 64);
    return __hiloint2double(hi, lo);
}

template <int NK>
__device__ __forceinline__ void scat2w_batch(const double* __restrict__ part, const size_t fq, const int q0, const int q1,
                                             const int qb, const int j, const int l, double (&S)[4])
{
    double v[4][NK];
#pragma unroll
    for (int m = 0; m < 4; ++m) {
#pragma unroll
        for (int k = 0; k < NK; ++k) {
            const int q = qb + j + 4 * m + 16 * k, qc = min(q, q1);
            const double t = part[((fq + qc) * 2 + (qc == q0 ? 1 : 0)) * SLOT + l];
            v[m][k] = q <= q1 ? t : 0.0;
        }
    }
#pragma unroll
    for (int m = 0; m < 4; ++m) {
#pragma unroll
        for (int k = 0; k < 4; ++k) S[m] += k < NK ? v[m][k] : 0.0;
    }
}

template <bool SHARED>
__device__ __forceinline__ void scat2w_form(const ScatArgs& sa, const int blk, const int nblk)
{
    const double* __restrict__ part = sa.part; const double* __restrict__ cpow = sa.cpow; const double lr = sa.lr;
    const int lane = threadIdx.x & 63, j = lane >> 4, l = lane & 15;
    const int gw = __builtin_amdgcn_readfirstlane(blk * 4 + ((int)threadIdx.x >> 6));
    const int NQ = sa.N2 >> 4, cap = sa.F * NQ;
    int4 ow = sa.owners[min(gw, cap - 1)];
    const int n = *sa.owner_cnt;
    for (int o = gw; o < n; o += 4 * nblk) {
        if (o != gw) ow = sa.owners[o];
        const int q0 = ow.y >> 4, q1 = (ow.z - 1) >> 4;
        const size_t fq = (size_t)ow.x * NQ;
        float* p = sa.table16 + (size_t)ow.w * SLOT + l;
        const float wold = *p;
        const double cdec = cpow[ow.z - ow.y];
        int mk = 0;
        if (SHARED) mk = sa.tag_shared[ow.w];
        double S[4] = {0.0, 0.0, 0.0, 0.0};
        if (q1 - q0 < 16) scat2w_batch<1>(part, fq, q0, q1, q0, j, l, S);
        else for (int qb = q0; qb <= q1; qb += 64) scat2w_batch<4>(part, fq, q0, q1, qb, j, l, S);
        double tot = 0.0;
#pragma unroll
        for (int g = 0; g < 16; ++g) tot += (g & 3) ? lane_from(S[g >> 2], (g & 3) * 16 + l) : S[g >> 2];
        if (SHARED && mk == sa.stamp) { if (j == 0 && l < sa.K) atomicAdd(p, (float)(-lr * tot)); }
        else if (j == 0 && l < sa.K) *p = (float)((double)wold * cdec - lr * tot);
    }
}
__device__ __forceinline__ void scat2w_body(const ScatArgs& sa, const int blk, const int nblk) { scat2w_form<false>(sa, blk, nblk); }
enum { SCAT2_BLOCK = 0, SCAT2_WAVE = 1 };
inline int scat2_form_env(const int dflt = SCAT2_WAVE)
{
    const char* e = getenv("FNN_SCAT2_FORM");
    if (!e) return dflt;
    return !strcmp(e, "block") ? SCAT2_BLOCK : !strcmp(e, "wave") ? SCAT2_WAVE : dflt;
}

static __global__ __launch_bounds__(256) void k_scat2(const ScatArgs sa)
{
    __shared__ double s_sum[16][16];
    if (sa.form2 == SCAT2_WAVE) scat2w_body(sa, blockIdx.x, gridDim.x);
    else scat2_body(sa, blockIdx.x, gridDim.x, s_sum);
}

constexpr int WCH = 32;

template <bool DECAY>
__device__ __forceinline__ void scatw1_form(const ScatArgs& sa, const int blk)
{
    const int rw = sa.rw, nq = rw >> 2, N2 = sa.N2, NQ = N2 / WCH;
    using gid_t = std::conditional_t<DECAY, int, long>;
    const gid_t gid = (gid_t)blk * 256 + (gid_t)threadIdx.x;
    const int chunk = (int)(gid / nq), q = (int)(gid % nq);
    if (chunk >= sa.F * NQ) return;
    const int f = chunk / NQ, qc = chunk % NQ, base = qc * WCH;
    const int lim = DECAY ? sa.K - 4 * q : 4;
    const double* __restrict__ cpow = sa.cpow; const double lr = sa.lr;
    double a0 = 0, a1 = 0, a2 = 0, a3 = 0;
    int4 rn[8];
#pragma unroll
    for (int j = 0; j < 8; ++j) rn[j] = sa.rec[(size_t)f * N2 + base + j];
    for (int sb = 0; sb < WCH; sb += 8) {
        int4 r[8];
#pragma unroll
        for (int j = 0; j < 8; ++j) r[j] = rn[j];
        if (r[0].x < 0) break;
        if (sb + 8 < WCH) {
#pragma unroll
            for (int j = 0; j < 8; ++j) rn[j] = sa.rec[(size_t)f * N2 + base + sb + 8 + j];
        }
        float4 g[8], wold[8];
        double wd[8], cs[8];
#pragma unroll
        for (int j = 0; j < 8; ++j) {
            const int pos = base + sb + j;
            const bool live = r[j].x >= 0;
// ... 85 lines not shown
            for (int gI = 0; gI < ngrp; ++gI) {
                const double* d = s_w + ((size_t)gI * nq + q) * 4;
                t0 += d[0]; t1 += d[1]; t2 += d[2]; t3 += d[3];
            }
            if constexpr (DECAY)
                *p = make_float4((float)((double)w.x * cdec - sa.lr * t0), (float)((double)w.y * cdec - sa.lr * t1),
                                 (float)((double)w.z * cdec - sa.lr * t2), (float)((double)w.w * cdec - sa.lr * t3));
            else if (sa.tag_shared[ow.w] == sa.stamp)
                atomic_add4(reinterpret_cast<float*>(p), (float)(-sa.lr * t0), (float)(-sa.lr * t1), (float)(-sa.lr * t2), (float)(-sa.lr * t3));
            else
                *p = make_float4((float)(w.x - sa.lr * t0), (float)(w.y - sa.lr * t1), (float)(w.z - sa.lr * t2),
                                 (float)(w.w - sa.lr * t3));
        }
        __syncthreads();
    }
}
__device__ __forceinline__ void scatw1_body(const ScatArgs& sa, const int blk) { scatw1_form<false>(sa, blk); }
__device__ __forceinline__ void scatw2_body(const ScatArgs& sa, const int blk, const int nblk, double* s_w) { scatw2_form<false>(sa, blk, nblk, s_w); }
__device__ __forceinline__ void scatdw1_body(const ScatArgs& sa, const int blk) { scatw1_form<true>(sa, blk); }
__device__ __forceinline__ void scatdw2_body(const ScatArgs& sa, const int blk, const int nblk, double* s_w) { scatw2_form<true>(sa, blk, nblk, s_w); }

static __global__ __launch_bounds__(256) void k_scatdw1(const ScatArgs sa) { scatdw1_body(sa, blockIdx.x); }
static __global__ __launch_bounds__(256) void k_scatdw2(const ScatArgs sa)
{
    __shared__ double s_w[1024];
    scatdw2_body(sa, blockIdx.x, gridDim.x, s_w);
}

struct RowGroupBufs { int4* rec = nullptr; double* part = nullptr; int4* owners = nullptr; int* owner_cnt = nullptr; };
inline hipError_t row_group_alloc(RowGroupBufs& b, int F, int N2, bool wide, int rw, hipStream_t st, bool owners16 = false)
{
    const size_t nchunk = (size_t)N2 / (wide ? WCH : 16);
    const size_t bytes[4] = {(size_t)F * N2 * sizeof(int4), (size_t)F * nchunk * 2 * rw * sizeof(double),
                             (size_t)F * (owners16 ? (size_t)N2 / 16 : nchunk) * sizeof(int4), sizeof(int)};
    void** const ptr[4] = {(void**)&b.rec, (void**)&b.part, (void**)&b.owners, (void**)&b.owner_cnt};
    for (int i = 0; i < 4; ++i) {
        hipError_t e = hipMalloc(ptr[i], bytes[i]);
        if (e == hipSuccess) e = hipMemsetAsync(*ptr[i], 0, bytes[i], st);
        if (e != hipSuccess) return e;
    }
    return hipSuccess;
}
inline void row_group_free(RowGroupBufs& b)
{
    for (void* p : {(void*)b.rec, (void*)b.part, (void*)b.owners, (void*)b.owner_cnt}) if (p) hipFree(p);
    b = RowGroupBufs();
}

inline ScatArgs scat_args(const RowGroupBufs& b, int N2, int F, int K, const float* gxp, int K1p, const double* cpow, double lr,
                          float* table, int rw)
{
    return ScatArgs{b.rec, N2, F, K, gxp, K1p, cpow, lr, table, b.part, b.owner_cnt, b.owners, rw,
                     nullptr,  0,  0,  SCAT1_QUARTER,  SCAT2_BLOCK};
}

template <int = 0> void launch_sort_runs(hipStream_t st, bool key64, const SortArgs& so)
{
    if (key64) hipLaunchKernelGGL((k_sortA<unsigned long long>), dim3(4 * so.F), dim3(256), sortA_lds_bytes<unsigned long long>(so.merge4), st, so);
    else hipLaunchKernelGGL((k_sortA<unsigned>), dim3(4 * so.F), dim3(256), sortA_lds_bytes<unsigned>(so.merge4), st, so);
}
template <int = 0> void launch_sort(hipStream_t st, bool key64, const SortArgs& so)
{
    launch_sort_runs(st, key64, so);
    if (key64) hipLaunchKernelGGL((k_sortB<unsigned long long>), dim3(16 * so.F), dim3(256), sort_lds_bytes<unsigned long long>(), st, so);
    else hipLaunchKernelGGL((k_sortB<unsigned>), dim3(16 * so.F), dim3(256), sort_lds_bytes<unsigned>(), st, so);
}
template <int = 0> void launch_k_sort(hipStream_t st, int N2, const int32_t* ids, int B, int F, int64_t n_rows, const RowGroupBufs& b,
                          const int32_t* extra, int n_extra, int* err)
{
    const int kpt = N2 <= 4096 ? 4 : (N2 == 8192 ? 8 : 16);
    const dim3 grid(F), blk(N2 / kpt);
    const size_t lds = (size_t)N2 * 8;
    if (kpt == 4) hipLaunchKernelGGL(k_sort<4>, grid, blk, lds, st, ids, B, F, n_rows, N2, b.rec, b.owner_cnt, extra, n_extra, err);
    else if (kpt == 8) hipLaunchKernelGGL(k_sort<8>, grid, blk, lds, st, ids, B, F, n_rows, N2, b.rec, b.owner_cnt, extra, n_extra, err);
    else hipLaunchKernelGGL(k_sort<16>, grid, blk, lds, st, ids, B, F, n_rows, N2, b.rec, b.owner_cnt, extra, n_extra, err);
}
inline void launch_scat_narrow(hipStream_t st, ScatArgs& sa, int form, int nblk2)
{
    const int nblk1 = scat1_blocks(sa, form);
    hipLaunchKernelGGL(k_scat1, dim3(nblk1), dim3(256), 0, st, sa);
    hipLaunchKernelGGL(k_scat2, dim3(nblk2), dim3(256), 0, st, sa);
}

}
```

include/fnn_hip.h:

```cpp
#ifndef FNN_HIP_H
#define FNN_HIP_H

#include <stdint.h>

#ifdef __cplusplus
extern "C" {
#endif
#if defined(__GNUC__)
#pragma GCC visibility push(default)
#endif

#define FNN_OK          0
#define FNN_ERR_ARG    -1
#define FNN_ERR_HIP    -2
#define FNN_ERR_STATE  -3
#define FNN_ERR_RANGE  -4
#define FNN_ERR_NOMEM  -5

#define FNN_PREC_F32    0
#define FNN_PREC_BF16   1
#define FNN_PREC_BF16X3 2

#define FNN_ACT_TANH    0
#define FNN_ACT_SIGMOID 1
#define FNN_ACT_LINEAR  2

#define FNN_MEM_HOST    0
#define FNN_MEM_DEVICE  1

#define FNN_MODE_FM     0
#define FNN_MODE_BAG    1

typedef struct fnn_cfg {
    int32_t n_fields;
    int32_t k;
    int32_t hidden1;
    int32_t hidden2;
    int32_t max_batch;
    int32_t precision;
    int32_t act;
    int32_t reg_all;
    float   lr;
    float   lambda1;
    float   lambda_fm;
    int32_t device;
    void*   stream;
    int32_t mode;
    int32_t h0;
} fnn_cfg;

typedef struct fnn_handle fnn_handle;

const char* fnn_version(void);
uint64_t fnn_cfg_size(void);
const char* fnn_last_error(const fnn_handle* h);
const char* fnn_scat1_form(void);
const char* fnn_scat2_form(void);

int fnn_create(const fnn_cfg* cfg, fnn_handle** out);
int fnn_destroy(fnn_handle* h);
int fnn_set_hparams(fnn_handle* h, float lr, float lambda1, float lambda_fm);
void* fnn_stream(fnn_handle* h);
int fnn_sync(fnn_handle* h);

int fnn_set_table(fnn_handle* h, const float* rows, int64_t n_rows,
                  const int32_t* field_of_row, float w0, int memkind);
int fnn_get_table(fnn_handle* h, float* rows_out, int memkind);
int fnn_get_rows(fnn_handle* h, const int64_t* row_ids, int64_t n, float* out, int memkind);

int fnn_set_dense(fnn_handle* h, int layer, const float* W, const float* b, int memkind);
int fnn_get_dense(fnn_handle* h, int layer, float* W, float* b, int memkind);

int fnn_set_bag_bias(fnn_handle* h, const float* bb0, int memkind);
int fnn_get_bag_bias(fnn_handle* h, float* bb0_out, int memkind);

int fnn_gather(fnn_handle* h, const int32_t* ids, int B, float* x_out, int memkind);

int fnn_train_step(fnn_handle* h, const int32_t* ids, const float* y, int B,
                   const uint8_t* mask1, const uint8_t* mask2, int b_size,
                   float* p_out, float* gx_out, int memkind, float* loss_sum_out);

int fnn_set_shadowed(fnn_handle* h, const int32_t* tfr, int n, int memkind);

int fnn_prefetch_ids(fnn_handle* h, const int32_t* ids, int B);

#define FNN_STEP_MAX_MODELS 256
int fnn_train_step_multi(fnn_handle* const* hs, int n_models, const int32_t* ids, const float* y, int B,
                         const uint8_t* const* mask1, const uint8_t* const* mask2, int b_size,
                         const int32_t* next_ids, int next_B, float* const* p_out, float* loss_sum_out);

// ... 53 lines not shown
```

Before: 145.3 million examples/sec.

## Split scatter owner list into per-field lists with padded counters

Replaces the single global owner list and counter, which every owner-producing thread appends to with an atomic, with one list and one counter per field. Each counter sits on its own padded stride so fields do not contend on the same cache line. The owner record is now emitted earlier from a per-chunk predicate, and scat2 waves are statically split across fields. This aims to cut atomic contention and serialization in the sparse embedding scatter, at the cost of possible load imbalance across fields and more kernel template variants.

Result: slower. 143.6 million examples/sec (-1.1%).

```diff
diff --git a/deep-ctr_amd/_capi.py b/deep-ctr_amd/_capi.py
--- a/deep-ctr_amd/_capi.py
+++ b/deep-ctr_amd/_capi.py
@@ -34,6 +34,7 @@
     "fnn_last_error": (C.c_char_p, [_vp]),
     "fnn_scat1_form": (C.c_char_p, []),
     "fnn_scat2_form": (C.c_char_p, []),
+    "fnn_owner_list": (C.c_char_p, []),
     "fnn_create": (_i, [C.POINTER(fnn_cfg), C.POINTER(_vp)]),
     "fnn_destroy": (_i, [_vp]),
     "fnn_set_hparams": (_i, [_vp, _f, _f, _f]),
diff --git a/deep-ctr_amd/csrc/fm_api.hip b/deep-ctr_amd/csrc/fm_api.hip
--- a/deep-ctr_amd/csrc/fm_api.hip
+++ b/deep-ctr_amd/csrc/fm_api.hip
@@ -325,6 +325,13 @@
     if (sa.form2 == SCAT2_WAVE) scat2w_body(sa, (int)blockIdx.x - 1, (int)gridDim.x - 1);
     else scat2_body(sa, (int)blockIdx.x - 1, (int)gridDim.x - 1, s_sum);
 }
+__global__ __launch_bounds__(256) void k_fm_scat2f_tail(const ScatArgs sa, float* b, const float* gb_part, int n, float lr, float lambda,
+                                                        const float* loss_t, int Ba, float lscale, float* loss_out, const FmBiasOpt bo)
+{
+    __shared__ float s_l[256];
+    if (blockIdx.x == 0) { fm_tail_body(b, gb_part, n, lr, lambda, loss_t, Ba, lscale, loss_out, s_l, bo); return; }
+    scat2wf_body(sa, (int)blockIdx.x - 1, (int)gridDim.x - 1);
+}
 __global__ __launch_bounds__(256) void k_fm_scat1s(const ScatArgs sa) { scat1h_form<true>(sa, blockIdx.x); }
 __global__ __launch_bounds__(256) void k_fm_scat2s_tail(const ScatArgs sa, float* b, const float* gb_part, int n, float lr, float lambda,
                                                         const float* loss_t, int Ba, float lscale, float* loss_out, const FmBiasOpt bo)
@@ -367,7 +374,7 @@
     const int lin = (int)blockIdx.x - ncls * mblk;
     m = args[first + lin / tiles].fcls;
     tile = lin % tiles;
-    if (tile == 0 && threadIdx.x == 0) *args[m].sa.owner_cnt = 0;
+    if (tile == 0) owner_cnt_clear(args[m].sa.owner_cnt, args[m].sa.F, threadIdx.x);
 }
 template <typename KT, int NF, bool WV>
 __global__ __launch_bounds__(256) void k_fm_step_fwd(const StepArg* __restrict__ args, const int ncls, const int mblk, const int first,
@@ -402,7 +409,7 @@
         if (r.x >= 0 && (i % sa.N2) == r.z && sa.tag_shared[r.x] == sa.stamp) g.own_marks[r.x] = g.own_stamp;
     }
 }
-template <bool SHARED>
+template <bool SHARED, bool OF = false>
 __global__ __launch_bounds__(256) void k_fm_step_scat1(const StepArg* __restrict__ args, const int first)
 {
     const int m = args[first + blockIdx.y].scls;
@@ -410,7 +417,8 @@
     if ((int)blockIdx.x >= nb1) return;
     const ScatArgs sa = args[m].sa;
     if (SHARED) step_copy_marks(args[m], sa, blockIdx.x, nb1);
-    scat1h_form<SHARED>(sa, blockIdx.x);
+    if (OF && !SHARED && sa.olist == OLIST_FIELD) scat1hf_body(sa, blockIdx.x);
+    else scat1h_form<SHARED>(sa, blockIdx.x);
 }
 __global__ __launch_bounds__(256) void k_fm_step_scatw1(const StepArg* __restrict__ args, const int first)
 {
@@ -431,14 +439,15 @@
         if (flag) *g.a.err = 0;
     }
 }
-template <bool SHARED>
+template <bool SHARED, bool OF = false>
 __global__ __launch_bounds__(256) void k_fm_step_scat2_tail(const StepArg* __restrict__ args, const int first)
 {
     __shared__ float s_l[256];
     const int m = args[first + blockIdx.y].scls;
     if (blockIdx.x == 0) { step_tail(args[m], s_l); return; }
     const ScatArgs sa = args[m].sa;
-    scat2w_form<SHARED>(sa, (int)blockIdx.x - 1, (int)gridDim.x - 1);
+    if (OF && !SHARED && sa.olist == OLIST_FIELD) scat2wf_body(sa, (int)blockIdx.x - 1, (int)gridDim.x - 1);
+    else scat2w_form<SHARED>(sa, (int)blockIdx.x - 1, (int)gridDim.x - 1);
 }
 __global__ __launch_bounds__(256) void k_fm_step_scatw2_tail(const StepArg* __restrict__ args, const int first)
 {
@@ -510,6 +519,7 @@
     int opt = FM_OPT_SGD; float beta1 = 0.9f, beta2 = 0.999f, eps = 1e-8f; int64_t t = 0; bool dense_g = false;
     int scat_form = SCAT1_HALF;
     int scat2_form = SCAT2_WAVE;
+    int owner_list = OLIST_FIELD;
     int sort_merge4 = 0;
     float *s0 = nullptr, *s1 = nullptr, *sb = nullptr, *G = nullptr; int* stamp = nullptr;
     bool shared = false; int* tag_first = nullptr; int* tag_shared = nullptr; int tag_stamp = 0, step_stamp = 0;
@@ -711,8 +721,9 @@
         p.sa.gxf = h->rw;
         p.nb1 = (F * (SORT_N / WCH) * (h->rw / 4) + 255) / 256;
     } else {
+        p.sa.form2 = form2;
+        p.sa.olist = h->shared ? OLIST_SINGLE : h->owner_list;
         p.nb1 = scat1_blocks(p.sa, form1);
-        p.sa.form2 = form2;
     }
     p.t = StepTail{h->b, h->gb_part, Ba / ex, lr, lambda, h->loss_t, Ba, dscale, h->loss_dev,
                    opt ? FmBiasOpt{h->opt, h->sb, p.lr_step, h->beta1, h->beta2, h->eps} : FmBiasOpt{FM_OPT_SGD, nullptr, 0.f, 0.f, 0.f, 0.f}};
@@ -739,6 +750,7 @@
                            t.loss_out, t.bo); } while (0)
     if (h->wide) FM_SCAT(k_fm_scatw1, k_fm_scatw2_tail);
     else if (h->shared) FM_SCAT(k_fm_scat1s, k_fm_scat2s_tail);
+    else if (p.sa.olist == OLIST_FIELD) FM_SCAT(k_scat1f, k_fm_scat2f_tail);
     else FM_SCAT(k_scat1, k_fm_scat2_tail);
 #undef FM_SCAT
     MHK(h, hipGetLastError());
@@ -868,6 +880,7 @@
     h->dense_g = getenv("FM_OPT_DENSE_G") && atoi(getenv("FM_OPT_DENSE_G")) == 1;
     h->scat_form = scat1_form_env();
     h->scat2_form = scat2_form_env();
+    h->owner_list = owner_list_env(h->owner_list);
     h->sort_merge4 = sort_merge4_env(0);
     if (const char* e = getenv("FM_ONLINE_CHUNK")) { const long long c = atoll(e); if (c >= 1) h->online_chunk = c; }
     *out = h;
@@ -1184,12 +1197,14 @@
     for (int c = 1; c < 3; ++c) { ffirst[c] = ffirst[c - 1] + fcnt[c - 1]; sfirst[c] = sfirst[c - 1] + scnt[c - 1]; }
     for (int c = 0; c < 3; ++c) { fpos[c] = ffirst[c]; spos[c] = sfirst[c]; }
     std::vector<float> lr_step(M);
+    bool by_field = false;
     for (int m = 0; m < M; ++m) {
         fm_handle* h = hs[m];
         const Cls& k = cls[cls_of[m]];
         const StepPlan p = plan_step(h, ids, wts, y, B, lr[m], lambda[m], reduce_mean ? reduce_mean[m] : 0, p_out ? p_out[m] : nullptr, wt,
                                      k.lead, k.stamp, SCAT1_HALF, SCAT2_WAVE);
         a[m].a = p.a; a[m].sa = p.sa; a[m].t = p.t; a[m].nb1 = p.nb1;
+        by_field = by_field || p.sa.olist == OLIST_FIELD;
         lr_step[m] = p.lr_step;
         a[m].own_marks = nullptr; a[m].own_stamp = 0;
         if (h->shared && h != k.lead) { a[m].own_marks = h->tag_shared; a[m].own_stamp = on_stream(h, st, [&] { return fm_next_stamp(h); }); }
@@ -1214,10 +1229,10 @@
         ride = 0;
     }
     MHK(h0, hipGetLastError());
-    if (scnt[0]) hipLaunchKernelGGL(k_fm_step_scat1<false>, dim3(nb1max[0], scnt[0]), dim3(256), 0, st, d, sfirst[0]);
+    if (scnt[0]) hipLaunchKernelGGL((by_field ? k_fm_step_scat1<false, true> : k_fm_step_scat1<false>), dim3(nb1max[0], scnt[0]), dim3(256), 0, st, d, sfirst[0]);
     if (scnt[1]) hipLaunchKernelGGL(k_fm_step_scat1<true>, dim3(nb1max[1], scnt[1]), dim3(256), 0, st, d, sfirst[1]);
     if (scnt[2]) hipLaunchKernelGGL(k_fm_step_scatw1, dim3(nb1max[2], scnt[2]), dim3(256), 0, st, d, sfirst[2]);
-    if (scnt[0]) hipLaunchKernelGGL(k_fm_step_scat2_tail<false>, dim3(1 + 256, scnt[0]), dim3(256), 0, st, d, sfirst[0]);
+    if (scnt[0]) hipLaunchKernelGGL((by_field ? k_fm_step_scat2_tail<false, true> : k_fm_step_scat2_tail<false>), dim3(1 + 256, scnt[0]), dim3(256), 0, st, d, sfirst[0]);
     if (scnt[1]) hipLaunchKernelGGL(k_fm_step_scat2_tail<true>, dim3(1 + 256, scnt[1]), dim3(256), 0, st, d, sfirst[1]);
     if (scnt[2]) hipLaunchKernelGGL(k_fm_step_scatw2_tail, dim3(1 + 256, scnt[2]), dim3(256), 0, st, d, sfirst[2]);
     MHK(h0, hipGetLastError());
diff --git a/deep-ctr_amd/csrc/fnn_api.hip b/deep-ctr_amd/csrc/fnn_api.hip
--- a/deep-ctr_amd/csrc/fnn_api.hip
+++ b/deep-ctr_amd/csrc/fnn_api.hip
@@ -17,6 +17,7 @@
 #include "fnn_step_kernels.hip.h"
 #include "metrics.hip.h"
 #include "arg_ring.h"
+static_assert(fnn::GROUP_OWNER_CNT_STRIDE == fnn::OWNER_CNT_STRIDE, "group_global clears the counters row_group_alloc lays out");
 
 using namespace fnn;
 
@@ -40,6 +41,7 @@
     int wgrad_form = -1;
     int scat_form = SCAT1_HALF;
     int scat2_form = SCAT2_WAVE;
+    int owner_list = -1;
     int sort_merge4 = 1;
 };
 
@@ -248,9 +250,11 @@
 int wgrad_blocks(const WgradArgs& wa) {
     return wa.p[0].mt * wa.p[0].nt + wa.p[1].mt * wa.p[1].nt + wa.p[2].mt * wa.p[2].nt + wa.p[3].mt * wa.p[3].nt;
 }
-ScatArgs make_scat_args(fnn_handle* h, const fnn_handle::SortSlot& sl, int N2) {
+int owner_list_of(const FnnKnobs& kn, bool three_launch) { return kn.owner_list >= 0 ? kn.owner_list : three_launch ? OLIST_FIELD : OLIST_SINGLE; }
+ScatArgs make_scat_args(fnn_handle* h, const fnn_handle::SortSlot& sl, int N2, bool three_launch = false) {
     ScatArgs sa = scat_args(sl, N2, h->F, h->K, h->gxp, h->K1p, h->cpow_dev, (double)h->cfg.lr, h->table16, h->rw);
     sa.tag_shared = sl.tag_shared; sa.stamp = sl.stamp; sa.form2 = h->kn.scat2_form;
+    sa.olist = owner_list_of(h->kn, three_launch);
     return sa;
 }
 template <typename T> MlpArgs<T> make_mlp_args(fnn_handle* h, const int32_t* ids, const float* y, int B,
@@ -278,21 +282,25 @@
     return big ? STEP1(5, 2, 4, false, 4) : STEP1(1, 1, 4, false, 4);
 #undef STEP1
 }
-template <typename T> Step2Kernel step2_sel(bool key64, bool m4, bool wgrad_lds)
-{
-#define STEP2(WF) (key64 ? (m4 ? Step2Kernel{k_step2<T, unsigned long long, true, WF>, 256, lds} : Step2Kernel{k_step2<T, unsigned long long, false, WF>, 256, lds}) \
-                         : (m4 ? Step2Kernel{k_step2<T, unsigned, true, WF>, 256, lds} : Step2Kernel{k_step2<T, unsigned, false, WF>, 256, lds}))
+template <typename T> Step2Kernel step2_sel(bool key64, bool m4, bool wgrad_lds, bool of)
+{
+#define STEP2K(KT, M4, WF) (of ? Step2Kernel{k_step2<T, KT, M4, WF, true>, 256, lds} : Step2Kernel{k_step2<T, KT, M4, WF>, 256, lds})
+#define STEP2(WF) (key64 ? (m4 ? STEP2K(unsigned long long, true, WF) : STEP2K(unsigned long long, false, WF)) \
+                         : (m4 ? STEP2K(unsigned, true, WF) : STEP2K(unsigned, false, WF)))
     const size_t lds = key64 ? sortA_lds_bytes<unsigned long long>(m4) : sortA_lds_bytes<unsigned>(m4);
     if constexpr (sizeof(T) == 2) if (wgrad_lds) return STEP2(WGRAD_LDS);
     return STEP2(WGRAD_DIRECT);
 #undef STEP2
-}
-template <typename T> Step3Kernel step3_sel(bool key64, bool m4, bool update)
-{
-#define STEP3(KT, LDS) (m4 ? (update ? Step3Kernel{k_step3<T, true, KT, true>, 256, LDS} : Step3Kernel{k_step3<T, false, KT, true>, 256, LDS}) \
-                           : (update ? Step3Kernel{k_step3<T, true, KT, false>, 256, LDS} : Step3Kernel{k_step3<T, false, KT, false>, 256, LDS}))
+#undef STEP2K
+}
+template <typename T> Step3Kernel step3_sel(bool key64, bool m4, bool update, bool of)
+{
+#define STEP3K(UP, KT, M4, LDS) (of ? Step3Kernel{k_step3<T, UP, KT, M4, true>, 256, LDS} : Step3Kernel{k_step3<T, UP, KT, M4>, 256, LDS})
+#define STEP3(KT, LDS) (m4 ? (update ? STEP3K(true, KT, true, LDS) : STEP3K(false, KT, true, LDS)) \
+                           : (update ? STEP3K(true, KT, false, LDS) : STEP3K(false, KT, false, LDS)))
     return key64 ? STEP3(unsigned long long, sort_lds_bytes<unsigned long long>()) : STEP3(unsigned, sort_lds_bytes<unsigned>());
 #undef STEP3
+#undef STEP3K
 }
 template <typename T> GroupKernel<T> gstep1_sel(const FnnPlan& p, const FnnKnobs& kn)
 {
@@ -314,21 +322,26 @@
     return big ? GPREDICT(5, 2, 4) : GPREDICT(1, 1, 4);
 #undef GPREDICT
 }
-template <typename T> GroupKernel<T> gstep2_sel(bool key64, bool m4, bool wgrad_lds)
-{
-#define GSTEP2(WF) (key64 ? (m4 ? GroupKernel<T>{k_gstep2<T, unsigned long long, true, WF>, 256, lds} : GroupKernel<T>{k_gstep2<T, unsigned long long, false, WF>, 256, lds}) \
-                          : (m4 ? GroupKernel<T>{k_gstep2<T, unsigned, true, WF>, 256, lds} : GroupKernel<T>{k_gstep2<T, unsigned, false, WF>, 256, lds}))
+template <typename T> GroupKernel<T> gstep2_sel(bool key64, bool m4, bool wgrad_lds, bool of)
+{
+#define GSTEP2K(KT, M4, WF) (of ? GroupKernel<T>{k_gstep2<T, KT, M4, WF, true>, 256, lds} : GroupKernel<T>{k_gstep2<T, KT, M4, WF>, 256, lds})
+#define GSTEP2(WF) (key64 ? (m4 ? GSTEP2K(unsigned long long, true, WF) : GSTEP2K(unsigned long long, false, WF)) \
+                          : (m4 ? GSTEP2K(unsigned, true, WF) : GSTEP2K(unsigned, false, WF)))
     const size_t lds = key64 ? sortA_lds_bytes<unsigned long long>(m4) : sortA_lds_bytes<unsigned>(m4);
     if constexpr (sizeof(T) == 2) if (wgrad_lds) return GSTEP2(WGRAD_LDS);
     return GSTEP2(WGRAD_DIRECT);
 #undef GSTEP2
-}
-template <typename T> GroupKernel<T> gstep3_sel(bool key64, bool m4)
-{
-#define GSTEP3(KT) (m4 ? GroupKernel<T>{k_gstep3<T, KT, true>, 256, sort_lds_bytes<KT>()} : GroupKernel<T>{k_gstep3<T, KT, false>, 256, sort_lds_bytes<KT>()})
+#undef GSTEP2K
+}
+template <typename T> GroupKernel<T> gstep3_sel(bool key64, bool m4, bool of)
+{
+#define GSTEP3K(KT, M4) (of ? GroupKernel<T>{k_gstep3<T, KT, M4, true>, 256, sort_lds_bytes<KT>()} : GroupKernel<T>{k_gstep3<T, KT, M4>, 256, sort_lds_bytes<KT>()})
+#define GSTEP3(KT) (m4 ? GSTEP3K(KT, true) : GSTEP3K(KT, false))
     return key64 ? GSTEP3(unsigned long long) : GSTEP3(unsigned);
 #undef GSTEP3
-}
+#undef GSTEP3K
+}
+bool owner_lists_by_field(const fnn_handle* h) { return owner_list_of(h->kn, true) == OLIST_FIELD && !h->bag && !h->wide; }
 template <typename T> void plan_step1(fnn_handle* h)
 {
     for (int train = 0; train < 2; ++train) {
@@ -340,8 +353,8 @@
 {
     h->key64 = key64;
     for (int i = 0; i < 2; ++i) {
-        h->step2[i] = step2_sel<T>(key64, h->kn.sort_merge4 != 0, i && h->wgrad_lds);
-        h->step3[i] = step3_sel<T>(key64, h->kn.sort_merge4 != 0, i != 0);
+        h->step2[i] = step2_sel<T>(key64, h->kn.sort_merge4 != 0, i && h->wgrad_lds, owner_lists_by_field(h));
+        h->step3[i] = step3_sel<T>(key64, h->kn.sort_merge4 != 0, i != 0, owner_lists_by_field(h));
     }
 }
 
@@ -365,8 +378,9 @@
 {
     const bool have_next = r.group_next && h->pend_have_next;
     fnn_handle::SortSlot& nx = h->slot[h->cur ^ 1];
-    Step23Args a{have_next, make_scat_args(h, h->slot[h->cur], SORT_N), {}};
+    Step23Args a{have_next, make_scat_args(h, h->slot[h->cur], SORT_N, true), {}};
     if (r.gxp_src) a.sa.gxp = r.gxp_src;
+    scat1_blocks(a.sa, h->kn.scat_form);
     a.so = SortArgs{h->next_ids, h->next_B, h->F, h->n_rows, nx.rec, nx.owner_cnt, have_next ? (merge ? 16 : 4) * h->F : 0, h->skeys,
                     merge ? h->tag_first : nullptr, merge ? nx.tag_shared : nullptr, merge && have_next ? next_stamp(h, nx) : 0, h->kn.sort_merge4};
     return a;
@@ -608,11 +622,11 @@
         ProfScope ps(h, "scatter", h->st);
         const int nblk = h->wide ? (int)(((size_t)h->F * (N2 / WCH) * (h->rw / 4) + 255) / 256) : scat1_blocks(sa, h->kn.scat_form);
         if (h->wide) hipLaunchKernelGGL(k_scatdw1, dim3(nblk), dim3(256), 0, h->st, sa);
-        else hipLaunchKernelGGL(k_scat1, dim3(nblk), dim3(256), 0, h->st, sa);
+        else hipLaunchKernelGGL(sa.olist == OLIST_FIELD ? k_scat1f : k_scat1, dim3(nblk), dim3(256), 0, h->st, sa);
     }
     ProfScope ps(h, "finalize", h->st);
     if (h->wide) hipLaunchKernelGGL(k_scatdw2, dim3(256), dim3(256), 0, h->st, sa);
-    else hipLaunchKernelGGL(k_scat2, dim3(64), dim3(256), 0, h->st, sa);
+    else hipLaunchKernelGGL(sa.olist == OLIST_FIELD ? k_scat2f : k_scat2, dim3(64), dim3(256), 0, h->st, sa);
 }
 
 template <typename T>
@@ -799,7 +813,7 @@
     if (const char* e = getenv("FNN_ROLE_OFF")) k.role_off = atoi(e);
     if (const char* e = getenv("FNN_SPLITK")) { const int v = atoi(e); if (v == 2 || v == 4 || v == 8 || v == 16) k.splitk = v; }
     if (const char* e = getenv("FNN_SCAT2_WGS")) { const int v = atoi(e); if (v >= 16 && v <= 1024) k.scat2_wgs = v; }
-    k.wgrad_form = wgrad_form_env(); k.scat_form = scat1_form_env(); k.scat2_form = scat2_form_env();
+    k.wgrad_form = wgrad_form_env(); k.scat_form = scat1_form_env(); k.scat2_form = scat2_form_env(); k.owner_list = owner_list_env(-1);
     k.sort_merge4 = sort_merge4_env(bag ? 0 : 1);
     return k;
 }
@@ -876,26 +890,26 @@
 }
 
 struct LaunchClass {
-    FnnKernel<> k[3]; int prec, F, K, K1p, H1p, H2p, splitk, wl, scat_form, scat2_form, scat2_wgs, wt_stores, role_off;
+    FnnKernel<> k[3]; int prec, F, K, K1p, H1p, H2p, splitk, wl, scat_form, scat2_form, owner_list, scat2_wgs, wt_stores, role_off;
     std::vector<int> members;
     bool same(const LaunchClass& o) const
     {
         for (int i = 0; i < 3; ++i) if (k[i].fn != o.k[i].fn || k[i].threads != o.k[i].threads || k[i].lds != o.k[i].lds) return false;
         return prec == o.prec && F == o.F && K == o.K && K1p == o.K1p && H1p == o.H1p && H2p == o.H2p && splitk == o.splitk && wl == o.wl &&
-               scat_form == o.scat_form && scat2_form == o.scat2_form && scat2_wgs == o.scat2_wgs && wt_stores == o.wt_stores && role_off == o.role_off;
+               scat_form == o.scat_form && scat2_form == o.scat2_form && owner_list == o.owner_list && scat2_wgs == o.scat2_wgs && wt_stores == o.wt_stores && role_off == o.role_off;
     }
 };
 template <typename T> LaunchClass launch_class_of(const fnn_handle* h)
 {
     const bool m4 = h->kn.sort_merge4 != 0;
     const bool wl = !(h->kn.role_off & 2) && h->wgrad_lds && sizeof(T) == 2;
-    const GroupKernel<T> k1 = gstep1_sel<T>(*h, h->kn), k2 = gstep2_sel<T>(h->key64, m4, wl), k3 = gstep3_sel<T>(h->key64, m4);
+    const GroupKernel<T> k1 = gstep1_sel<T>(*h, h->kn), k2 = gstep2_sel<T>(h->key64, m4, wl, owner_lists_by_field(h)), k3 = gstep3_sel<T>(h->key64, m4, owner_lists_by_field(h));
     LaunchClass c{};
     c.k[0] = {reinterpret_cast<void (*)()>(k1.fn), k1.threads, k1.lds};
     c.k[1] = {reinterpret_cast<void (*)()>(k2.fn), k2.threads, std::max(k2.lds, wl ? WGRAD_LDS_BYTES : (size_t)0)};
     c.k[2] = {reinterpret_cast<void (*)()>(k3.fn), k3.threads, k3.lds};
     c.prec = h->cfg.precision; c.F = h->F; c.K = h->K; c.K1p = h->K1p; c.H1p = h->H1p; c.H2p = h->H2p; c.splitk = h->splitk; c.wl = wl;
-    c.scat_form = h->kn.scat_form; c.scat2_form = h->kn.scat2_form; c.scat2_wgs = h->kn.scat2_wgs; c.wt_stores = h->kn.wt_stores;
+    c.scat_form = h->kn.scat_form; c.scat2_form = h->kn.scat2_form; c.owner_list = owner_list_of(h->kn, true); c.scat2_wgs = h->kn.scat2_wgs; c.wt_stores = h->kn.wt_stores;
     c.role_off = h->kn.role_off;
     return c;
 }
@@ -1079,6 +1093,12 @@
 {
     const int f = scat2_form_env(-1);
     return f == SCAT2_BLOCK ? "block" : f == SCAT2_WAVE ? "wave" : "default";
+}
+
+const char* fnn_owner_list(void)
+{
+    const int o = owner_list_env(-1);
+    return o == OLIST_SINGLE ? "single" : o == OLIST_FIELD ? "field" : "default";
 }
 
 const char* fnn_scat1_form(void)
diff --git a/deep-ctr_amd/csrc/fnn_step_kernels.hip.h b/deep-ctr_amd/csrc/fnn_step_kernels.hip.h
--- a/deep-ctr_amd/csrc/fnn_step_kernels.hip.h
+++ b/deep-ctr_amd/csrc/fnn_step_kernels.hip.h
@@ -20,15 +20,17 @@
     }
     wgrad_body<T, WF>(wa, w % nwx, w / nwx, smem);
 }
+template <bool OF = false>
 __device__ __forceinline__ void scat1_role(const ScatArgs& sa, const int blk)
 {
     if (sa.rw != SLOT) scatw1_body(sa, blk);
+    else if (OF && sa.form == SCAT1_HALF && sa.olist == OLIST_FIELD) scat1hf_body(sa, blk);
     else if (sa.form == SCAT1_SLOT) scat1_body(sa, blk);
     else if (sa.form == SCAT1_HALF) scat1h_body(sa, blk);
     else scat1q_body(sa, blk);
 }
 
-template <typename T, typename KT, bool M4, int WF = WGRAD_DIRECT>
+template <typename T, typename KT, bool M4, int WF = WGRAD_DIRECT, bool OF = false>
 static __global__ __launch_bounds__(256) void k_step2(const SortArgs so, const WgradArgs wa, const int nwx,
                                                const int splitk, const ScatArgs sa)
 {
@@ -41,6 +43,7 @@
     }
     else if (sa.rw != SLOT) scatw1_body(sa, b - so.nblk - nw);
     else if (sa.form == SCAT1_SLOT) scat1_body(sa, b - so.nblk - nw);
+    else if (OF && sa.form == SCAT1_HALF && sa.olist == OLIST_FIELD) scat1hf_body(sa, b - so.nblk - nw);
     else if (sa.form == SCAT1_HALF) scat1h_body(sa, b - so.nblk - nw);
     else scat1q_body(sa, b - so.nblk - nw);
 }
@@ -122,16 +125,18 @@
         ta.master[i] = w - ta.lr * g;
     }
 }
+template <bool OF = false>
 __device__ __forceinline__ void scat2_role(const ScatArgs& sa, const int blk, const int nb, double (*s_sum)[16], unsigned char* smem)
 {
     if (sa.rw == SLOT) {
-        if (sa.form2 == SCAT2_WAVE) scat2w_body(sa, blk, nb);
+        if (OF && sa.form2 == SCAT2_WAVE && sa.olist == OLIST_FIELD) scat2wf_body(sa, blk, nb);
+        else if (sa.form2 == SCAT2_WAVE) scat2w_body(sa, blk, nb);
         else scat2_body(sa, blk, nb, s_sum);
     }
     else scatw2_body(sa, blk, nb, reinterpret_cast<double*>(smem));
 }
 
-template <typename T, bool UPDATE, typename KT, bool M4>
+template <typename T, bool UPDATE, typename KT, bool M4, bool OF = false>
 static __global__ __launch_bounds__(256) void k_step3(const SortArgs so, const TailArgs ta, const ScatArgs sa)
 {
     extern __shared__ __align__(16) unsigned char smem[];
@@ -141,7 +146,8 @@
     if (b >= ta.nblk_red) {
         const int nb = (int)gridDim.x - so.nblk - ta.nblk_red;
         if (sa.rw == SLOT) {
-            if (sa.form2 == SCAT2_WAVE) scat2w_body(sa, b - ta.nblk_red, nb);
+            if (OF && sa.form2 == SCAT2_WAVE && sa.olist == OLIST_FIELD) scat2wf_body(sa, b - ta.nblk_red, nb);
+            else if (sa.form2 == SCAT2_WAVE) scat2w_body(sa, b - ta.nblk_red, nb);
             else scat2_body(sa, b - ta.nblk_red, nb, s_sum);
         }
         else scatw2_body(sa, b - ta.nblk_red, nb, reinterpret_cast<double*>(smem));
@@ -168,12 +174,13 @@
     const MlpArgs<T> a = g.ma;
     const int nmlp = g.nmlp;
     int* const owner_cnt = g.sa.owner_cnt;
+    const int F = g.sa.F;
     if ((int)blockIdx.x >= nmlp) return;
-    if (blockIdx.x == 0 && threadIdx.x == 0) *owner_cnt = 0;
+    if (blockIdx.x == 0) owner_cnt_clear(owner_cnt, F, threadIdx.x);
     mlp_body<T, C1, C2, CX, false, NW, WTF>(a, blockIdx.x, smem);
 }
 
-template <typename T, typename KT, bool M4, int WF>
+template <typename T, typename KT, bool M4, int WF, bool OF = false>
 static __global__ __launch_bounds__(256) void k_gstep2(const GroupArg<T>* __restrict__ args)
 {
     extern __shared__ __align__(16) unsigned char smem[];
@@ -185,10 +192,10 @@
         const int w = b - nsort;
         wgrad_role<T, WF>(wa, nwx, w, nw, ((b ^ w) & 7) == 0, smem);
     }
-    else if (b < nsort + nw + nsc) { const ScatArgs sa = g.sa; scat1_role(sa, b - nsort - nw); }
-}
-
-template <typename T, typename KT, bool M4>
+    else if (b < nsort + nw + nsc) { const ScatArgs sa = g.sa; scat1_role<OF>(sa, b - nsort - nw); }
+}
+
+template <typename T, typename KT, bool M4, bool OF = false>
 static __global__ __launch_bounds__(256) void k_gstep3(const GroupArg<T>* __restrict__ args)
 {
     extern __shared__ __align__(16) unsigned char smem[];
@@ -198,7 +205,7 @@
     if ((int)blockIdx.x < nsort) { const SortArgs so = g.so3; sortB_form<KT, M4>(so, blockIdx.x, smem); return; }
     const int b = (int)blockIdx.x - nsort;
     if (b >= nred) {
-        if (b - nred < nsc) { const ScatArgs sa = g.sa; scat2_role(sa, b - nred, nsc, s_sum, smem); }
+        if (b - nred < nsc) { const ScatArgs sa = g.sa; scat2_role<OF>(sa, b - nred, nsc, s_sum, smem); }
         return;
     }
     const TailArgs ta = g.ta;
diff --git a/deep-ctr_amd/csrc/ipnn_api.hip b/deep-ctr_amd/csrc/ipnn_api.hip
--- a/deep-ctr_amd/csrc/ipnn_api.hip
+++ b/deep-ctr_amd/csrc/ipnn_api.hip
@@ -1358,7 +1358,7 @@
     bool wt = true;
     int group_wgrad = 1, group_xcd = 1;
     int wgrad_want = 0;
-    int scat_form = SCAT1_HALF, scat2_form = SCAT2_WAVE, sort_merge4 = 1;
+    int scat_form = SCAT1_HALF, scat2_form = SCAT2_WAVE, sort_merge4 = 1, owner_list = OLIST_FIELD;
     int stamps = 0, stamp_sel = -1;
 };
 
@@ -1459,7 +1459,7 @@
     int nf = 4, nw = 8;
     if (getenv("IPNN_WIDE") && sscanf(getenv("IPNN_WIDE"), "%d:%d", &nf, &nw) == 2 && ((nf == 2 && (nw == 8 || nw == 12)) || (nf == 4 && nw == 8))) { k.wide_nf = nf; k.wide_nw = nw; }
     k.wgrad_want = getenv("IPNN_WGRAD_WANT") ? std::max(16, env_int("IPNN_WGRAD_WANT", 0)) : k.group_wgrad ? 144 : 288;
-    k.scat_form = scat1_form_env(); k.scat2_form = scat2_form_env(); k.sort_merge4 = sort_merge4_env(1);
+    k.scat_form = scat1_form_env(); k.scat2_form = scat2_form_env(); k.sort_merge4 = sort_merge4_env(1); k.owner_list = owner_list_env(k.owner_list);
     if (getenv("IPNN_STAMPS")) k.stamps = env_int("IPNN_STAMPS", 0) == 2 ? 2 : 1;
     return k;
 }
@@ -1928,7 +1928,7 @@
             hipLaunchKernelGGL(k_ip_scatw1, dim3((nthr + 255) / 256), dim3(256), 0, ss, sa);
             hipLaunchKernelGGL(k_ip_scatw2, dim3(256), dim3(256), 0, ss, sa);
         } else {
-            sa.form2 = h->kn.scat2_form;
+            sa.form2 = h->kn.scat2_form; sa.olist = h->kn.owner_list;
             launch_scat_narrow(ss, sa, h->kn.scat_form, 256);
         }
     }
diff --git a/deep-ctr_amd/csrc/metrics.hip b/deep-ctr_amd/csrc/metrics.hip
--- a/deep-ctr_amd/csrc/metrics.hip
+++ b/deep-ctr_amd/csrc/metrics.hip
@@ -212,7 +212,7 @@
                                                     unsigned long long* __restrict__ keys, int* __restrict__ owner_cnt)
 {
     const size_t gid = (size_t)blockIdx.x * 256 + threadIdx.x;
-    if (gid == 0) *owner_cnt = 0;
+    if (gid < F) owner_cnt[(size_t)gid * GROUP_OWNER_CNT_STRIDE] = 0;
     if (gid >= (size_t)F * N2) return;
     const int f = (int)(gid / N2), t = (int)(gid % N2);
     unsigned long long row = G_INV;
diff --git a/deep-ctr_amd/csrc/metrics.hip.h b/deep-ctr_amd/csrc/metrics.hip.h
--- a/deep-ctr_amd/csrc/metrics.hip.h
+++ b/deep-ctr_amd/csrc/metrics.hip.h
@@ -6,6 +6,7 @@
 namespace fnn {
 int device_metrics(hipStream_t st, const float* p, const int32_t* y, int64_t n, double out[4], std::string& err);
 
+constexpr int GROUP_OWNER_CNT_STRIDE = 32;
 int group_global(hipStream_t st, const int32_t* ids, int B, int F, int64_t n_rows, int N2, int4* rec, int* owner_cnt,
                  void** ws, size_t* ws_bytes, std::string& err);
 
diff --git a/deep-ctr_amd/csrc/sparse_rows.hip.h b/deep-ctr_amd/csrc/sparse_rows.hip.h
--- a/deep-ctr_amd/csrc/sparse_rows.hip.h
+++ b/deep-ctr_amd/csrc/sparse_rows.hip.h
@@ -6,6 +6,12 @@
 template <typename KT> struct KeyTraits;
 template <> struct KeyTraits<unsigned> { static constexpr int SH = 12; };
 template <> struct KeyTraits<unsigned long long> { static constexpr int SH = 32; };
+
+constexpr int OWNER_CNT_STRIDE = 32;
+__device__ __forceinline__ void owner_cnt_clear(int* __restrict__ cnt, const int F, const int tid)
+{
+    if (tid < F) cnt[tid * OWNER_CNT_STRIDE] = 0;
+}
 
 struct SortArgs {
     const int32_t* ids; int B, F; int64_t n_rows; int4* rec; int* owner_cnt; int nblk; void* skeys;
@@ -124,7 +130,7 @@
     constexpr int SH = KeyTraits<KT>::SH;
     KT* s_key = reinterpret_cast<KT*>(smem);
     const int tid = threadIdx.x, f = blk >> 4, run = blk & 15;
-    if (blk == 0 && tid == 0) *so.owner_cnt = 0;
+    if (blk == 0) owner_cnt_clear(so.owner_cnt, so.F, tid);
     const KT* in = static_cast<const KT*>(so.skeys) + (size_t)f * SORT_N;
 #pragma unroll
     for (int a = 0; a < 16; ++a) s_key[a * 256 + tid] = in[a * 256 + tid];
@@ -215,7 +221,7 @@
     extern __shared__ unsigned long long s_key[];
     __shared__ int s_cnt;
     const int f = blockIdx.x, tid = threadIdx.x;
-    if (f == 0 && tid == 0) *owner_cnt = 0;
+    if (f == 0) owner_cnt_clear(owner_cnt, F, tid);
     int cnt = 0;
     if (n_extra > 0) {
         if (tid == 0) s_cnt = 0;
@@ -316,7 +322,10 @@
     int gxf;
     int form;
     int form2;
+    int olist;
 };
+enum { SCAT2_BLOCK = 0, SCAT2_WAVE = 1 };
+enum { OLIST_SINGLE = 0, OLIST_FIELD = 1 };
 enum { SCAT1_QUARTER = 0, SCAT1_SLOT = 1, SCAT1_HALF = 2 };
 __device__ __forceinline__ void atomic_add4(float* p, float a, float b, float c, float d) {
     atomicAdd(p, a); atomicAdd(p + 1, b); atomicAdd(p + 2, c); atomicAdd(p + 3, d);
@@ -444,7 +453,7 @@
     return __hiloint2double(hi, lo);
 }
 
-template <bool SHARED>
+template <bool SHARED, bool OF = false>
 __device__ __forceinline__ void scat1h_form(const ScatArgs& sa, const int blk)
 {
     const int N2 = sa.N2, NQ = N2 >> 4, nq = (sa.K + 3) >> 2;
@@ -458,6 +467,9 @@
     int4 r[8];
 #pragma unroll
     for (int j = 0; j < 8; ++j) r[j] = sa.rec[(size_t)f * N2 + hb + j];
+    const bool reg = OF && half && q == 0 && r[7].x >= 0 && r[7].z >= base && r[7].w > base + 16;
+    int oi = 0;
+    if (OF && reg) oi = atomicAdd(sa.owner_cnt + (size_t)f * OWNER_CNT_STRIDE, 1);
     float4 g[8], wold[8];
     double wd[8], cs[8];
     int mk[8];
@@ -487,6 +499,7 @@
         a0 += (double)g[j].x * wd[j]; a1 += (double)g[j].y * wd[j]; a2 += (double)g[j].z * wd[j]; a3 += (double)g[j].w * wd[j];
         if (hb + j + 1 == r[j].w) a0 = a1 = a2 = a3 = 0;
     }
+    if (OF && reg && oi < NQ) sa.owners[(size_t)f * NQ + oi] = make_int4(f, r[7].z, r[7].w, r[7].x);
     a0 = lane_below(a0); a1 = lane_below(a1); a2 = lane_below(a2); a3 = lane_below(a3);
     if (!half) a0 = a1 = a2 = a3 = 0;
 #pragma unroll
@@ -510,12 +523,13 @@
             const int which = (s < base) ? 0 : 1;
             double* pp = sa.part + (((size_t)f * NQ + qc) * 2 + which) * SLOT + 4 * q;
             pp[0] = a0; pp[1] = a1; pp[2] = a2; pp[3] = a3;
-            if (which == 1 && q == 0) sa.owners[atomicAdd(sa.owner_cnt, 1)] = make_int4(f, s, e, r[j].x);
+            if (!OF && which == 1 && q == 0) sa.owners[atomicAdd(sa.owner_cnt, 1)] = make_int4(f, s, e, r[j].x);
         }
         a0 = a1 = a2 = a3 = 0;
     }
 }
 __device__ __forceinline__ void scat1h_body(const ScatArgs& sa, const int blk) { scat1h_form<false>(sa, blk); }
+__device__ __forceinline__ void scat1hf_body(const ScatArgs& sa, const int blk) { scat1h_form<false, true>(sa, blk); }
 
 static __global__ __launch_bounds__(256) void k_scat1(const ScatArgs sa)
 {
@@ -523,11 +537,13 @@
     else if (sa.form == SCAT1_HALF) scat1h_body(sa, blockIdx.x);
     else scat1q_body(sa, blockIdx.x);
 }
+static __global__ __launch_bounds__(256) void k_scat1f(const ScatArgs sa) { scat1hf_body(sa, blockIdx.x); }
 
 inline int scat1_blocks(ScatArgs& sa, const int form)
 {
     const bool vec_ok = ((uintptr_t)sa.gxp | (uintptr_t)sa.table16) % 16 == 0 && sa.K1p % 4 == 0;
     sa.form = vec_ok ? form : SCAT1_SLOT;
+    if (sa.form != SCAT1_HALF || sa.form2 != SCAT2_WAVE || sa.rw != SLOT) sa.olist = OLIST_SINGLE;
     const size_t nquarters = (size_t)sa.F * (sa.N2 / 16) * ((sa.K + 3) / 4);
     const size_t nthr = sa.form == SCAT1_SLOT ? (size_t)sa.F * sa.N2 : sa.form == SCAT1_HALF ? 2 * nquarters : nquarters;
     return (int)((nthr + 255) / 256);
@@ -603,17 +619,21 @@
     }
 }
 
-template <bool SHARED>
+template <bool SHARED, bool OF = false>
 __device__ __forceinline__ void scat2w_form(const ScatArgs& sa, const int blk, const int nblk)
 {
     const double* __restrict__ part = sa.part; const double* __restrict__ cpow = sa.cpow; const double lr = sa.lr;
     const int lane = threadIdx.x & 63, j = lane >> 4, l = lane & 15;
     const int gw = __builtin_amdgcn_readfirstlane(blk * 4 + ((int)threadIdx.x >> 6));
-    const int NQ = sa.N2 >> 4, cap = sa.F * NQ;
-    int4 ow = sa.owners[min(gw, cap - 1)];
-    const int n = *sa.owner_cnt;
-    for (int o = gw; o < n; o += 4 * nblk) {
-        if (o != gw) ow = sa.owners[o];
+    const int NQ = sa.N2 >> 4, cap = OF ? NQ : sa.F * NQ;
+    const int per = OF ? (4 * nblk) / sa.F : 0;
+    const int o0 = OF ? gw / sa.F : gw, step = OF ? per : 4 * nblk;
+    if (OF && o0 >= per) return;
+    const int4* list = OF ? sa.owners + (size_t)(gw % sa.F) * NQ : sa.owners;
+    int4 ow = list[min(o0, cap - 1)];
+    const int n = OF ? min(sa.owner_cnt[(size_t)(gw % sa.F) * OWNER_CNT_STRIDE], NQ) : *sa.owner_cnt;
+    for (int o = o0; o < n; o += step) {
+        if (o != o0) ow = list[o];
         const int q0 = ow.y >> 4, q1 = (ow.z - 1) >> 4;
         const size_t fq = (size_t)ow.x * NQ;
         float* p = sa.table16 + (size_t)ow.w * SLOT + l;
@@ -632,7 +652,13 @@
     }
 }
 __device__ __forceinline__ void scat2w_body(const ScatArgs& sa, const int blk, const int nblk) { scat2w_form<false>(sa, blk, nblk); }
-enum { SCAT2_BLOCK = 0, SCAT2_WAVE = 1 };
+__device__ __forceinline__ void scat2wf_body(const ScatArgs& sa, const int blk, const int nblk) { scat2w_form<false, true>(sa, blk, nblk); }
+inline int owner_list_env(const int dflt)
+{
+    const char* e = getenv("FNN_OWNER_LIST");
+    if (!e) return dflt;
+    return !strcmp(e, "single") ? OLIST_SINGLE : !strcmp(e, "field") ? OLIST_FIELD : dflt;
+}
 inline int scat2_form_env(const int dflt = SCAT2_WAVE)
 {
     const char* e = getenv("FNN_SCAT2_FORM");
@@ -646,6 +672,7 @@
     if (sa.form2 == SCAT2_WAVE) scat2w_body(sa, blockIdx.x, gridDim.x);
     else scat2_body(sa, blockIdx.x, gridDim.x, s_sum);
 }
+static __global__ __launch_bounds__(256) void k_scat2f(const ScatArgs sa) { scat2wf_body(sa, blockIdx.x, gridDim.x); }
 
 constexpr int WCH = 32;
 
@@ -797,7 +824,7 @@
 {
     const size_t nchunk = (size_t)N2 / (wide ? WCH : 16);
     const size_t bytes[4] = {(size_t)F * N2 * sizeof(int4), (size_t)F * nchunk * 2 * rw * sizeof(double),
-                             (size_t)F * (owners16 ? (size_t)N2 / 16 : nchunk) * sizeof(int4), sizeof(int)};
+                             (size_t)F * (owners16 ? (size_t)N2 / 16 : nchunk) * sizeof(int4), (size_t)F * OWNER_CNT_STRIDE * sizeof(int)};
     void** const ptr[4] = {(void**)&b.rec, (void**)&b.part, (void**)&b.owners, (void**)&b.owner_cnt};
     for (int i = 0; i < 4; ++i) {
         hipError_t e = hipMalloc(ptr[i], bytes[i]);
@@ -816,7 +843,7 @@
                           float* table, int rw)
 {
     return ScatArgs{b.rec, N2, F, K, gxp, K1p, cpow, lr, table, b.part, b.owner_cnt, b.owners, rw,
-                     nullptr,  0,  0,  SCAT1_QUARTER,  SCAT2_BLOCK};
+                     nullptr,  0,  0,  SCAT1_QUARTER,  SCAT2_BLOCK,  OLIST_SINGLE};
 }
 
 template <int = 0> void launch_sort_runs(hipStream_t st, bool key64, const SortArgs& so)
@@ -843,8 +870,8 @@
 inline void launch_scat_narrow(hipStream_t st, ScatArgs& sa, int form, int nblk2)
 {
     const int nblk1 = scat1_blocks(sa, form);
-    hipLaunchKernelGGL(k_scat1, dim3(nblk1), dim3(256), 0, st, sa);
-    hipLaunchKernelGGL(k_scat2, dim3(nblk2), dim3(256), 0, st, sa);
-}
-
-}
+    hipLaunchKernelGGL(sa.olist == OLIST_FIELD ? k_scat1f : k_scat1, dim3(nblk1), dim3(256), 0, st, sa);
+    hipLaunchKernelGGL(sa.olist == OLIST_FIELD ? k_scat2f : k_scat2, dim3(nblk2), dim3(256), 0, st, sa);
+}
+
+}
diff --git a/include/fnn_hip.h b/include/fnn_hip.h
--- a/include/fnn_hip.h
+++ b/include/fnn_hip.h
@@ -56,6 +56,7 @@
 const char* fnn_last_error(const fnn_handle* h);
 const char* fnn_scat1_form(void);
 const char* fnn_scat2_form(void);
+const char* fnn_owner_list(void);
 
 int fnn_create(const fnn_cfg* cfg, fnn_handle** out);
 int fnn_destroy(fnn_handle* h);
```
